# microsoft/OmniParser

Hardware: AMD Instinct MI355X
Metric: screenshots/sec end-to-end (detect+caption) @1920x1080 (higher is better)
Workload: dtype f32 (split-f16x3 MFMA)

## Files before the change

include/omni_amd.h:

```cpp
#ifndef OMNI_AMD_H
#define OMNI_AMD_H

#include <stdint.h>
#include <stddef.h>

#ifdef __cplusplus
extern "C" {
#endif

#define OMNI_ABI_VERSION 3

enum { OMNI_F32 = 0, OMNI_F16 = 1 };
enum { OMNI_ACT_NONE = 0, OMNI_ACT_SILU = 1, OMNI_ACT_GELU = 2 };
enum {
  OMNI_OK = 0,
  OMNI_E_ARG = -1,
  OMNI_E_HIP = -2,
  OMNI_E_NODEV = -3
};

const char* omni_last_error(void);
int omni_abi_version(void);
int omni_device_count(void);
int omni_overflow_count(int reset, unsigned long long* count);

typedef struct omni_op {
  int32_t kind;
  int32_t dtype;
  void*   p[8];
  int32_t i[32];
  float   f[8];
} omni_op_t;

enum {
  OMNI_OP_CONV = 1,
  OMNI_OP_AVGPOOL2 = 2,
  OMNI_OP_MAXPOOL = 3,
  OMNI_OP_RESIZE_NEAREST = 4,
  OMNI_OP_LETTERBOX = 5,
  OMNI_OP_DETECT_DECODE = 6,
  OMNI_OP_NMS = 7,
  OMNI_OP_DWCONV3 = 8,
  OMNI_OP_LAYERNORM = 9,
  OMNI_OP_ATTN_ROWS = 10,
  OMNI_OP_CHAN_ATTN = 11,
  OMNI_OP_PROJ_PREP = 12,
  OMNI_OP_ASSEMBLE = 13,
  OMNI_OP_EMBED_STEP = 14,
  OMNI_OP_ATTN_DECODE = 15,
  OMNI_OP_GREEDY_STEP = 16,
  OMNI_OP_CROP_RESIZE = 17,
  OMNI_OP_DWCONV3_LN = 18,
  OMNI_OP_SPLIT_CONVERT = 19,
  OMNI_OP_GLUE = 20,
  OMNI_OP_OVERLAY = 21,
  OMNI_OP_PNG_PACK = 22,
  OMNI_OP_PNG_DEFLATE = 23,
  OMNI_OP_MLP_FUSED = 24,
  OMNI_OP_BEAM_STEP,
  OMNI_OP__COUNT,
  OMNI_OP_GREEDY_CTRL_STEP = OMNI_OP__COUNT,
  OMNI_OP_GREEDY_VOCAB_STEP = OMNI_OP_GREEDY_CTRL_STEP + 1,
  OMNI_OP_VISUAL_MATCH = OMNI_OP_GREEDY_VOCAB_STEP + 1,
  OMNI_OP_REGION_OCR = OMNI_OP_VISUAL_MATCH + 1,
  OMNI_OP__END
};

#define OMNI_OCR_CLASS_STRIP 1000
#define OMNI_OCR_CLASS_TEXT 1001
#define OMNI_OCR_CLASS_HARD 1002

#define OMNI_VOCAB_HEADER_BYTES 32
#define OMNI_VOCAB_MAX_NODES 65536
#define OMNI_VOCAB_MAX_LABEL 64
typedef struct omni_vocab_trie {
  int32_t n_nodes;
  int32_t n_edges;
  int32_t longest;
  int32_t reserved[5];
} omni_vocab_trie_t;

#define OMNI_GEN_CTRL_HEADER_BYTES 32
#define OMNI_GEN_CTRL_MAX_BAD 64
#define OMNI_GEN_CTRL_MAX_BAD_LEN 8
typedef struct omni_gen_ctrl {
  float penalty;
  int32_t ngram;
  int32_t min_new_tokens;
  int32_t begin_index;
  int32_t n_bad;
  int32_t bad_stride;
  int32_t reserved[2];
} omni_gen_ctrl_t;

typedef struct omni_cand {
  float x1, y1, x2, y2;
  float score;
  int32_t cls;
  int32_t anchor;
  int32_t pad;
} omni_cand_t;

int omni_op_launch(const omni_op_t* op, void* stream);

typedef struct omni_plan omni_plan_t;
int omni_plan_create(const omni_op_t* ops, int n_ops, omni_plan_t** out);
int omni_plan_run(omni_plan_t* plan, void* stream);
int omni_plan_capture(omni_plan_t* plan, void* stream);
int omni_plan_replay(omni_plan_t* plan, void* stream);
int omni_plan_num_ops(const omni_plan_t* plan);
void omni_plan_destroy(omni_plan_t* plan);

int omni_resample_coeffs(int in_size, int out_size, int filter, int32_t* h_bounds, int32_t* h_coef);

int omni_plan_time(omni_plan_t* plan, void* stream, int iters, float* ms);

int omni_plan_profile(omni_plan_t* plan, void* stream, float* h_ms);

int omni_debug_tile_map(int mtiles, int ntiles, int xcd_n, long long weight_bytes, int bid, int* mt, int* nt, int* grid,
// ... 27 lines not shown
```

omniparser_amd/_lib.py:

```python
import ctypes
from ctypes import c_char_p, c_float, c_int, c_int32, c_void_p, POINTER, Structure

from . import build as _build


F32, F16 = 0, 1
ACT_NONE, ACT_SILU, ACT_GELU = 0, 1, 2
OP_CONV, OP_AVGPOOL2, OP_MAXPOOL, OP_RESIZE_NEAREST, OP_LETTERBOX, OP_DETECT_DECODE, OP_NMS = 1, 2, 3, 4, 5, 6, 7
OP_DWCONV3, OP_LAYERNORM, OP_ATTN_ROWS, OP_CHAN_ATTN, OP_PROJ_PREP, OP_ASSEMBLE = 8, 9, 10, 11, 12, 13
OP_EMBED_STEP, OP_ATTN_DECODE, OP_GREEDY_STEP, OP_CROP_RESIZE, OP_DWCONV3_LN, OP_SPLIT_CONVERT, OP_GLUE = 14, 15, 16, 17, 18, 19, 20
OP_OVERLAY, OP_PNG_PACK, OP_PNG_DEFLATE, OP_MLP_FUSED, OP_BEAM_STEP = 21, 22, 23, 24, 25
OP_GREEDY_CTRL_STEP = 26
OP_GREEDY_VOCAB_STEP = 27
OP_VISUAL_MATCH = 28
OP_REGION_OCR = 29
OCR_CLASS_STRIP, OCR_CLASS_TEXT, OCR_CLASS_HARD = 1000, 1001, 1002
CAND_BYTES = 32
ABI_VERSION = 3

EXPORTS = [
    "omni_last_error", "omni_abi_version", "omni_device_count", "omni_op_launch",
    "omni_plan_create", "omni_plan_run", "omni_plan_capture", "omni_plan_replay",
    "omni_plan_num_ops", "omni_plan_destroy", "omni_resample_coeffs", "omni_plan_time", "omni_debug_tile_map",
    "omni_debug_conv_cfg",
    "omni_plan_profile",
    "omni_model_load", "omni_model_destroy", "omni_model_int", "omni_model_tensor", "omni_model_run",
    "omni_detector_create", "omni_detector_infer", "omni_captioner_create", "omni_captioner_caption",
    "omni_overflow_count",
    "omni_visual_match_cfg",
]


class OmniOp(Structure):
    _fields_ = [
        ("kind", c_int32),
        ("dtype", c_int32),
        ("p", c_void_p * 8),
        ("i", c_int32 * 32),
        ("f", c_float * 8),
    ]


class OmniError(RuntimeError):
    pass


_lib = None


def lib():
    global _lib
    if _lib is not None:
        return _lib
    path = _build.ensure_built()
    import torch
    _lib = bind(path)
    return _lib


def bind(path):
    L = ctypes.CDLL(str(path))
    missing = [s for s in EXPORTS if not hasattr(L, s)]
    if missing:
        raise OmniError(f"{path} does not export {missing}")
    L.omni_last_error.restype = c_char_p
    L.omni_abi_version.restype = c_int
    L.omni_device_count.restype = c_int
    L.omni_op_launch.argtypes = [POINTER(OmniOp), c_void_p]
# ... 268 lines not shown
```

omniparser_amd/bundle.py:

```python
import bisect
import struct
from typing import Dict

import numpy as np
import torch

from . import _lib as L
from . import planner

MAGIC = b"OMNIPLN%d" % L.ABI_VERSION
ROLE = {"scratch": 0, "zero": 1, "const": 2}


def _name(s: str) -> bytes:
    b = s.encode()
    assert len(b) < 32, s
    return b.ljust(32, b"\0")


def f32_bits(x: float) -> int:
    return struct.unpack("<i", struct.pack("<f", float(x)))[0]


def write_bundle(path, plans: Dict[str, list], named: Dict[str, tuple], ints: Dict[str, int]):
# ... 88 lines not shown
        ops = []
        for _ in range(n):
            kind, dtype = struct.unpack_from("<ii", b, p); p += 8
            ptrs = [struct.unpack_from("<iq", b, p + 12 * j) for j in range(8)]; p += 96
            ii = struct.unpack_from("<32i", b, p); p += 128
            ff = struct.unpack_from("<8f", b, p); p += 32
            ops.append((kind, dtype, ptrs, ii, ff))
        plans[nm] = ops
    named = {}
    for _ in range(nn):
        nm = b[p:p + 32].rstrip(b"\0").decode(); p += 32
        named[nm] = struct.unpack_from("<iqq", b, p); p += 20
    ints = {}
    for _ in range(ni):
        nm = b[p:p + 32].rstrip(b"\0").decode(); p += 32
        (ints[nm],) = struct.unpack_from("<q", b, p); p += 8
    return {"tensors": tensors, "plans": plans, "named": named, "ints": ints}


def export_detector(det, iw: int, ih: int, path, imgsz=640, conf=0.05, iou=0.1, max_det=300, batch=1):
    dp = det.get_plan(iw, ih, imgsz, conf, iou, max_det, batch=batch)
    t = lambda x: (x, 0, x.numel() * x.element_size())
    named = {"img": t(dp.img), "out_boxes": t(dp.out_boxes), "out_scores": t(dp.out_scores), "out_cls": t(dp.out_cls),
             "out_count": t(dp.out_count)}
    ints = {"model": 1, "batch": batch, "img_w": iw, "img_h": ih, "max_det": max_det, "dtype": det.dtype}
    return write_bundle(path, {"detect": dp.plan.ops}, named, ints)


def export_captioner(cap, path, capacity=8, max_new_tokens=20):
    from .florence import CLIP_MEAN, CLIP_STD
    R = cap.resolution
    cp = cap.plans(capacity, R, max_new_tokens)
    pb = planner.PlanBuilder(cap.device, cap.dtype)
    lut = pb.upload(torch.from_numpy((np.arange(256).astype(np.float64) * (1 / 255)).astype(np.float32)))
    boxes = pb.raw((capacity, 4), torch.int32)
    c64 = pb.raw((capacity, 64, 64, 3), torch.uint8)
    t = lambda x: (x, 0, x.numel() * x.element_size())
    named = {"x_in": t(cp.x_in.t), "ids": t(cp.ids), "finished": t(cp.finished), "step": t(cp.step), "lut": t(lut), "boxes": t(boxes),
             "c64": t(c64),
             "vision_out": t(cp.vision_out.t), "enc_out": t(cp.enc_out.t), "logits": t(cp.logits.t)}
    ks = 0
    if R != 64:
        b, k = L.resample_coeffs(64, R, 1)
        bb, kk = pb.upload(torch.from_numpy(b)), pb.upload(torch.from_numpy(k))
        tmp = pb.raw((capacity, 64, R, 3), torch.uint8)
        named.update(bic_bounds=t(bb), bic_coef=t(kk), tmp=t(tmp))
        ks = k.shape[1]
    cp._bundle_keep = pb.keep
    ints = {"model": 2, "capacity": capacity, "R": R, "T": cp.T, "max_new": max_new_tokens, "start_token": cp.start_token, "pad": cap.w.pad,
            "eos": cap.w.eos, "ksize": ks, "ldo": cp.x_in.ld, "dtype": cap.dtype}
    for j in range(3):
        ints[f"mean{j}"] = f32_bits(CLIP_MEAN[j])
        ints[f"std{j}"] = f32_bits(CLIP_STD[j])
    return write_bundle(path, {"encode": cp.encode_plan.ops, "step": cp.step_plan.ops}, named, ints)
```

omniparser_amd/csrc/capi.hip:

```cpp
#include "omni_internal.h"

#include <math.h>
#include <stdarg.h>
#include <stdlib.h>
#include <string.h>
#include <vector>

static thread_local char g_err[512] = "";

void omni_set_error(const char* fmt, ...) {
  va_list ap;
  va_start(ap, fmt);
  vsnprintf(g_err, sizeof(g_err), fmt, ap);
  va_end(ap);
}

extern "C" const char* omni_last_error(void) { return g_err; }
extern "C" int omni_abi_version(void) { return OMNI_ABI_VERSION; }

static omni_ovf_reader_t g_ovf_readers[8];
static int g_ovf_n = 0;
void omni_register_overflow_reader(omni_ovf_reader_t fn) {
  if (g_ovf_n < 8) g_ovf_readers[g_ovf_n++] = fn;
}
extern "C" int omni_overflow_count(int reset, unsigned long long* count) {
  OMNI_REQUIRE(count != nullptr, "omni_overflow_count: null result pointer");
  unsigned long long total = 0;
  for (int k = 0; k < g_ovf_n; ++k) {
    unsigned int v = 0;
    if (g_ovf_readers[k](&v, reset)) {
      omni_set_error("omni_overflow_count: reading the device counter failed");
      return OMNI_E_HIP;
    }
    total += v;
  }
  *count = total;
  return OMNI_OK;
}

extern "C" int omni_device_count(void) {
  int n = 0;
  hipError_t e = hipGetDeviceCount(&n);
  if (e != hipSuccess) {
    omni_set_error("hipGetDeviceCount: %s", hipGetErrorString(e));
    return OMNI_E_NODEV;
  }
  return n;
}

static int dispatch(const omni_op_t* op, hipStream_t s) {
  switch (op->kind) {
    case OMNI_OP_CONV: return op->i[20] == 2 ? omni_launch_gemm_dma(op, s) : omni_launch_conv(op, s);
    case OMNI_OP_SPLIT_CONVERT: return omni_launch_split_convert(op, s);
    case OMNI_OP_MLP_FUSED: return omni_launch_mlp_fused(op, s);
    case OMNI_OP_GLUE: return omni_launch_glue(op, s);
    case OMNI_OP_OVERLAY: return omni_launch_overlay(op, s);
    case OMNI_OP_PNG_PACK: return omni_launch_png_pack(op, s);
    case OMNI_OP_PNG_DEFLATE: return omni_launch_png_deflate(op, s);
    case OMNI_OP_AVGPOOL2: return omni_launch_avgpool2(op, s);
    case OMNI_OP_MAXPOOL: return omni_launch_maxpool(op, s);
    case OMNI_OP_RESIZE_NEAREST: return omni_launch_resize_nearest(op, s);
    case OMNI_OP_LETTERBOX: return omni_launch_letterbox(op, s);
    case OMNI_OP_DETECT_DECODE: return omni_launch_detect_decode(op, s);
    case OMNI_OP_NMS: return omni_launch_nms(op, s);
    case OMNI_OP_DWCONV3: return omni_launch_dwconv3(op, s);
    case OMNI_OP_LAYERNORM: return omni_launch_layernorm(op, s);
    case OMNI_OP_DWCONV3_LN: return omni_launch_dwconv3_ln(op, s);
    case OMNI_OP_ATTN_ROWS: case OMNI_OP_CHAN_ATTN: case OMNI_OP_ATTN_DECODE: return omni_launch_attention(op, s);
    case OMNI_OP_PROJ_PREP: case OMNI_OP_ASSEMBLE: case OMNI_OP_EMBED_STEP: case OMNI_OP_GREEDY_STEP:
    case OMNI_OP_BEAM_STEP: case OMNI_OP_GREEDY_CTRL_STEP: case OMNI_OP_CROP_RESIZE: return omni_launch_misc(op, s);
    case OMNI_OP_GREEDY_VOCAB_STEP: return omni_launch_vocab_step(op, s);
    case OMNI_OP_VISUAL_MATCH: return omni_launch_visual_match(op, s);
    case OMNI_OP_REGION_OCR: return omni_launch_region_ocr(op, s);
    default:
      omni_set_error("unknown op kind %d", op->kind);
      return OMNI_E_ARG;
  }
}

static bool check_ptrs_enabled() {
  const char* e = getenv("OMNI_CHECK_PTRS");
  if (e && e[0] == '0') return false;
  static const int ndev = [] { int n = 0; const bool ok = hipGetDeviceCount(&n) == hipSuccess; if (!ok) (void)hipGetLastError(); return ok ? n : 0; }();
  return ndev > 0;
}

static void op_extents(const omni_op_t* op, long long ext[8]) {
  for (int k = 0; k < 8; ++k) ext[k] = 1;
  const long long esz = op->dtype == OMNI_F32 ? 4 : 2;
  const int* i = op->i;
  auto span = [&](long long rows, long long ld, long long coff, long long c) { return rows > 0 ? ((rows - 1) * ld + coff + c) * esz : 1; };
  switch (op->kind) {
    case OMNI_OP_CONV: {
      const long long B = i[0], H = i[1], W = i[2], Cin = i[3], Cout = i[12], M = B * i[10] * i[11], K = (long long)i[6] * i[7] * Cin;
      ext[0] = span(B * H * W, i[4], i[5], i[25] ? i[4] : Cin);
      ext[1] = Cout * K * (i[20] ? 4 : esz);
      ext[2] = Cout * 4;
      ext[3] = span(M, i[16], i[17], Cout);
      ext[4] = span(M, i[13], i[14], Cout);
      ext[5] = i[19] > 0 ? (long long)i[19] * 1024 : 1;
      if (i[24] > 0) ext[6] = (long long)i[24] * 4;
      if (i[20] == 2 && i[26] > 0) {
        const long long nimg = (M + i[26] - 1) / i[26];
        ext[1] += (nimg - 1) * (long long)i[27];
        ext[6] = nimg * 4;
        if (i[29] == 1) ext[2] = nimg * Cout * 4;
      }
      if (i[20] == 2 && i[28] == 1) {
        ext[7] = (M / 256) * (Cout / 64) * 4096;
        ext[4] = 1;
      }
      break;
    }
    case OMNI_OP_CHAN_ATTN: {
      const long long B = i[0], N = i[1], C = i[3], G = i[4], ct = i[10] > 0 ? i[10] : (i[5] > 0 ? i[5] : 1);
      ext[0] = B * N * 3 * C * esz; ext[4] = B * N * C * esz; ext[5] = B * G * ((N + ct - 1) / ct) * 1024 * 4;
      if (i[8] == 1) { ext[1] = C * C * 4; ext[2] = ext[3] = B * C * C * 4; ext[6] = B * 4; ext[7] = B * (C / 64) * G * 4; }
      if (i[8] == 1 && i[11] == 1) { ext[1] += 2 * C * 4; ext[2] += B * C * 4; }
      break;
    }
    case OMNI_OP_BEAM_STEP: {
      const long long rows = (long long)i[0] * i[6], T = i[3];
      ext[0] = rows > 0 ? ((rows - 1) * i[2] + i[1]) * esz : 1;
      ext[1] = (long long)i[1] * 4;
      ext[2] = ext[4] = ext[5] = rows * T * 4;
      ext[3] = rows * 4;
      ext[7] = (long long)i[0] * (3LL * i[6] + 2) * 4;
      break;
    }
    case OMNI_OP_GREEDY_STEP:
      if (op->p[5] || op->p[7]) {
        const long long rows = i[0], T = i[3];
        ext[0] = rows > 0 ? ((rows - 1) * i[2] + i[1]) * esz : 1;
        ext[1] = (long long)i[1] * 4;
        ext[2] = ext[4] = ext[7] = rows * T * 4;
        ext[5] = rows * 4;
        ext[6] = 4;
      }
      break;
    case OMNI_OP_GREEDY_CTRL_STEP: {
      const long long rows = i[0], T = i[3];
      ext[0] = rows > 0 ? ((rows - 1) * i[2] + i[1]) * esz : 1;
      ext[1] = (long long)i[1] * 4;
      ext[2] = ext[4] = rows * T * 4;
      ext[3] = rows * 4;
      ext[6] = 4;
      ext[7] = i[12];
      break;
    }
    case OMNI_OP_GREEDY_VOCAB_STEP: {
      const long long rows = i[0], T = i[3];
      ext[0] = rows > 0 ? ((rows - 1) * i[2] + i[1]) * esz : 1;
      ext[1] = (long long)i[1] * 4;
      ext[2] = ext[4] = rows * T * 4;
      ext[3] = ext[5] = rows * 4;
      ext[6] = 4;
      ext[7] = i[12];
      break;
    }
    case OMNI_OP_VISUAL_MATCH: {
      const long long D = i[3];
      if (i[0] == 0) {
        ext[0] = i[1] > 0 ? (((long long)i[1] - 1) * i[2] + D) * esz : 1; ext[4] = (long long)i[1] * D * 4; ext[5] = (long long)i[1] * 4;
      } else if (const long long part = omni_visual_match_part_bytes(op)) {
        ext[5] = part;
        if (i[0] == 1) { ext[0] = (long long)i[1] * D * 4; ext[1] = (long long)i[2] * D * 4; }
// ... 40 lines not shown
      break;
    }
    case OMNI_OP_DETECT_DECODE: {
      for (int l = 0; l < 3; ++l) {
        const long long hw = (long long)(i[1] / (8 << l)) * (i[2] / (8 << l));
        ext[l] = span(hw, i[3 + l], i[13 + l], i[0]);
        ext[3 + l] = span(hw, i[6 + l], i[16 + l], i[12] ? 4 : 64);
      }
      ext[6] = (long long)i[9] * 32; ext[7] = 4;
      break;
    }
    case OMNI_OP_LAYERNORM: {
      const long long rows = (long long)i[0] * i[1], C = i[3];
      ext[0] = rows * C * esz; ext[1] = (long long)(i[5] > 0 ? i[5] : 1) * C * esz; ext[2] = C * 4; ext[3] = C * 4;
      ext[4] = rows * C * esz; ext[5] = rows * C * esz;
      break;
    }
    case OMNI_OP_DWCONV3: case OMNI_OP_DWCONV3_LN: {
      const long long n = (long long)i[0] * i[1] * i[2] * i[3] * esz, C = i[3];
      ext[0] = n; ext[1] = 9 * C * esz; ext[2] = C * 4; ext[4] = n;
      if (op->kind == OMNI_OP_DWCONV3_LN) { ext[3] = n; ext[5] = C * 4; ext[6] = C * 4; }
      break;
    }
    case OMNI_OP_ASSEMBLE: {
      const long long B = i[0], n_img = i[1], n_txt = i[2], C = i[3];
      ext[0] = B * n_img * C * esz; ext[1] = n_txt * C * esz; ext[2] = B * n_txt * 4; ext[3] = (long long)i[4] * C * esz;
      ext[4] = B * (n_img + n_txt) * C * esz;
      break;
    }
    case OMNI_OP_ATTN_ROWS:
      ext[7] = (long long)i[11] * 4;
      break;
    case OMNI_OP_ATTN_DECODE:
      ext[7] = i[7] > 0 ? (long long)((i[10] + (i[12] > 1 ? i[12] : 1) - 1) / (i[12] > 1 ? i[12] : 1)) * 4 : (long long)i[10] * i[8] * 4;
      break;
    case OMNI_OP_OVERLAY:
      if (op->p[3] || op->p[4] || i[3]) {
        const long long B = i[3] > 0 ? i[3] : 1;
        ext[0] = B * i[0] * i[1] * 3; ext[1] = (long long)i[2] * 32; ext[3] = B * 8; ext[4] = (B + 1) * 4;
      }
      break;
    case OMNI_OP_PNG_DEFLATE:
      if (i[5] == 2 && i[6] > 0 && i[0] > 0 && i[1] > 0) {
        const long long B = i[6], U = (long long)i[0] * (3LL * i[1] + 1), units = (U + 32767) / 32768;
        ext[0] = B * i[0] * i[1] * 3; ext[1] = B * i[2]; ext[2] = B * U; ext[3] = B * units * 33792; ext[4] = B * i[3] * 4;
        ext[5] = B * i[4] * 4; ext[6] = B * 4 * (((long long)i[2] + 2) / 3); ext[7] = B * units * 32768 * 4;
      }
      break;
    default: break;
  }
  for (int k = 0; k < 8; ++k) if (ext[k] < 1) ext[k] = 1;
}

static int check_op_ptrs(const omni_op_t* op, int index) {
  long long ext[8];
  op_extents(op, ext);
  for (int k = 0; k < 8; ++k) {
    const void* ptr = op->p[k];
    if (!ptr) continue;
    hipDeviceptr_t base = nullptr;
    size_t size = 0;
    hipError_t e = hipMemGetAddressRange(&base, &size, (hipDeviceptr_t)ptr);
    if (e != hipSuccess || !base) {
      (void)hipGetLastError();
      omni_set_error("op %d (kind %d): p[%d] = %p is not inside any device allocation (%s)", index, op->kind, k, ptr,
                     e != hipSuccess ? hipGetErrorString(e) : "no base");
      return OMNI_E_ARG;
    }
    const long long off = (const char*)ptr - (const char*)base;
    if (off < 0 || off + ext[k] > (long long)size) {
      omni_set_error("op %d (kind %d): p[%d] = %p + %lld bytes runs past its allocation [%p, +%zu)", index, op->kind, k, ptr, ext[k],
                     (void*)base, size);
      return OMNI_E_ARG;
    }
  }
  return OMNI_OK;
}

static int check_ctrl_block(const omni_op_t* op, int index) {
  if (op->kind != OMNI_OP_GREEDY_CTRL_STEP) return OMNI_OK;
  const long long bytes = op->i[12], nw = ((long long)op->i[1] + 31) >> 5, fixed = OMNI_GEN_CTRL_HEADER_BYTES + 8 * nw;
  if (!op->p[7] || op->i[1] <= 0 || bytes < fixed) {
    omni_set_error("op %d (greedy_ctrl_step): a control block of %lld bytes (i12) at p7 = %p cannot hold the header and two bitmaps over a "
                   "vocabulary of %d (%lld bytes)", index, bytes, op->p[7], op->i[1], fixed);
    return OMNI_E_ARG;
  }
  omni_gen_ctrl_t h;
  hipError_t e = hipMemcpy(&h, op->p[7], sizeof h, hipMemcpyDeviceToHost);
  if (e != hipSuccess) {
    (void)hipGetLastError();
    omni_set_error("op %d (greedy_ctrl_step): the header of the control block p7 = %p cannot be read (%s)", index, op->p[7], hipGetErrorString(e));
    return OMNI_E_ARG;
  }
  if (h.n_bad < 0 || h.n_bad > OMNI_GEN_CTRL_MAX_BAD || (h.n_bad > 0 && (h.bad_stride < 3 || h.bad_stride > OMNI_GEN_CTRL_MAX_BAD_LEN + 1))) {
    omni_set_error("op %d (greedy_ctrl_step): the control block claims %d bad-word sequences of stride %d (at most %d of 2..%d tokens)", index,
                   h.n_bad, h.bad_stride, OMNI_GEN_CTRL_MAX_BAD, OMNI_GEN_CTRL_MAX_BAD_LEN);
    return OMNI_E_ARG;
  }
  const long long need = fixed + 4LL * h.n_bad * h.bad_stride;
  if (bytes < need) {
    omni_set_error("op %d (greedy_ctrl_step): the control block's header claims %d bad-word sequences of stride %d = %lld bytes, i12 says %lld",
                   index, h.n_bad, h.bad_stride, need, bytes);
    return OMNI_E_ARG;
  }
  return OMNI_OK;
}

static int check_trie_block(const omni_op_t* op, int index) {
  if (op->kind != OMNI_OP_GREEDY_VOCAB_STEP) return OMNI_OK;
  const long long bytes = op->i[12];
  if (!op->p[7] || bytes < OMNI_VOCAB_HEADER_BYTES + 4) {
    omni_set_error("op %d (greedy_vocab_step): a trie block of %lld bytes (i12) at p7 = %p cannot hold the header and one node (%d bytes)",
                   index, bytes, op->p[7], OMNI_VOCAB_HEADER_BYTES + 4);
    return OMNI_E_ARG;
  }
  omni_vocab_trie_t h;
  hipError_t e = hipMemcpy(&h, op->p[7], sizeof h, hipMemcpyDeviceToHost);
  if (e != hipSuccess) {
    (void)hipGetLastError();
    omni_set_error("op %d (greedy_vocab_step): the header of the trie block p7 = %p cannot be read (%s)", index, op->p[7], hipGetErrorString(e));
    return OMNI_E_ARG;
  }
  if (h.n_nodes < 1 || h.n_nodes > OMNI_VOCAB_MAX_NODES || h.n_edges < 0 || h.n_edges >= h.n_nodes) {
    omni_set_error("op %d (greedy_vocab_step): the trie block claims %d nodes and %d edges (1..%d nodes, fewer edges than nodes)", index,
                   h.n_nodes, h.n_edges, OMNI_VOCAB_MAX_NODES);
    return OMNI_E_ARG;
  }
  const long long need = OMNI_VOCAB_HEADER_BYTES + 4LL * (h.n_nodes + 1 + 2LL * h.n_edges);
// ... 192 lines not shown
```

omniparser_amd/csrc/conv_igemm.hip:

```cpp
#include "omni_internal.h"
#include "gemm_common.h"
#include <stdlib.h>
#include <string.h>
#include <type_traits>

OMNI_RANGE_GUARD_TU()

namespace {

struct ConvArgs {
  const void* x; const void* w; const float* bias; const void* res; void* y;
  int B, H, W, Cin, ldi, in_coff, KH, KW, stride, pad, Ho, Wo;
  int Cout, ldo, out_coff, act, ldr, res_coff;
  int M, K, ktiles, cin_tiles;
  int splits, kt_per_split, mtiles, ntiles, xcd_order, xcd_n;
  float* ws;
  int* cnt;
  float scale;
  int vec_px;
};


template <typename T, int ACT, typename GetAcc>
__device__ __forceinline__ void epilogue_tile(const ConvArgs& a, int mb, int n, bool nok, float bias, GetAcc get) {
  if (!nok) return;
  T* __restrict__ Yb = reinterpret_cast<T*>(a.y) + (long long)mb * a.ldo + a.out_coff + n;
  const T* __restrict__ Rb = a.res ? reinterpret_cast<const T*>(a.res) + (long long)mb * a.ldr + a.res_coff + n : nullptr;
  float r[16];
#pragma unroll
  for (int e = 0; e < 16; ++e) {
    const int dm = (e & 3) + 8 * (e >> 2);
    r[e] = (Rb && mb + dm < a.M) ? ElemTraits<T>::to_f32(Rb[dm * a.ldr]) : 0.0f;
  }
  const float scale = a.scale;
  float amax = 0.0f;
#pragma unroll
  for (int e = 0; e < 16; ++e) {
    const int dm = (e & 3) + 8 * (e >> 2);
    float v = get(e) + bias;
    if (scale != 0.0f) v *= scale;
    if constexpr (ACT == OMNI_ACT_SILU) v = v / (1.0f + expf(-v));
    else if constexpr (ACT == OMNI_ACT_GELU) v = omni_gelu(v);
    v += r[e];
    if (mb + dm < a.M) {
      Yb[dm * a.ldo] = ElemTraits<T>::from_f32(v);
      amax = __builtin_fmaxf(__builtin_fabsf(v), amax);
    }
  }
  if constexpr (sizeof(T) == 4) omni_report_range(amax);
}

template <typename T, int BM, int BN, int RB, bool ALIGNED, bool PW>
__global__ __launch_bounds__(256) void conv_igemm_kernel(ConvArgs a) {
  constexpr int V = ElemTraits<T>::kVec;
  constexpr int VPR = RB / 16;
  constexpr int BKE = VPR * V;
  constexpr int ROWB = RB + 16;
  constexpr int RPP = 256 / VPR;
  constexpr int A_IT = BM / RPP;
  constexpr int B_IT = BN / RPP;
  constexpr int TM = BM / 64;
  constexpr int TN = BN / 64;
  constexpr int STAGE = (BM + BN) * ROWB;

  __shared__ __attribute__((aligned(16))) unsigned char lds[2 * STAGE];

  const int tid = threadIdx.x;
  const int lane = tid & 63;
  const int wave = tid >> 6;
  const int wm = wave >> 1, wn = wave & 1;
  int mt, nt;
  if (!tile_of_block(blockIdx.x, a.mtiles, a.ntiles, a.xcd_order, a.xcd_n, mt, nt)) return;
// ... 219 lines not shown
  if constexpr (sizeof(T) == 4) omni_report_range(__builtin_fabsf(v));
  reinterpret_cast<T*>(a.y)[m * a.ldo + a.out_coff + n] = ElemTraits<T>::from_f32(v);
}


__device__ __forceinline__ void split_f16x4(const u32x4& raw, uint2& hi, uint2& lo) {
  typedef __fp16 hv2 __attribute__((ext_vector_type(2)));
  f32x4 v = __builtin_bit_cast(f32x4, raw);
  hv2 h01 = __builtin_amdgcn_cvt_pkrtz(v[0], v[1]);
  hv2 h23 = __builtin_amdgcn_cvt_pkrtz(v[2], v[3]);
  float r0 = (v[0] - (float)h01[0]) * 2048.0f, r1 = (v[1] - (float)h01[1]) * 2048.0f;
  float r2 = (v[2] - (float)h23[0]) * 2048.0f, r3 = (v[3] - (float)h23[1]) * 2048.0f;
  hv2 l01 = __builtin_amdgcn_cvt_pkrtz(r0, r1);
  hv2 l23 = __builtin_amdgcn_cvt_pkrtz(r2, r3);
  hi.x = __builtin_bit_cast(unsigned, h01); hi.y = __builtin_bit_cast(unsigned, h23);
  lo.x = __builtin_bit_cast(unsigned, l01); lo.y = __builtin_bit_cast(unsigned, l23);
}

#ifndef OMNI_AGENT_ST_F32
#define OMNI_AGENT_ST_F32(p, v) __hip_atomic_store((p), (v), __ATOMIC_RELAXED, __HIP_MEMORY_SCOPE_AGENT)
#define OMNI_AGENT_LD_F32(p) __hip_atomic_load((p), __ATOMIC_RELAXED, __HIP_MEMORY_SCOPE_AGENT)
#define OMNI_AGENT_ADD_I32(p, v) __hip_atomic_fetch_add((p), (v), __ATOMIC_RELAXED, __HIP_MEMORY_SCOPE_AGENT)
#define OMNI_AGENT_ST_I32(p, v) __hip_atomic_store((p), (v), __ATOMIC_RELAXED, __HIP_MEMORY_SCOPE_AGENT)
#endif

__device__ __forceinline__ void combine_partials(const ConvArgs& a, int mb, int n, bool nok, float* sum) {
#pragma unroll
  for (int e = 0; e < 16; ++e) sum[e] = 0.0f;
  if (!nok) return;
  const int total = a.M * a.Cout;
  int off[16];
#pragma unroll
  for (int e = 0; e < 16; ++e) {
    const int m = mb + (e & 3) + 8 * (e >> 2);
    off[e] = (m < a.M ? m : a.M - 1) * a.Cout + n;
  }
  const float* __restrict__ base = a.ws;
  int z = 0;
  for (; z + 2 <= a.splits; z += 2, base += 2 * (long long)total) {
    float v0[16], v1[16];
#pragma unroll
    for (int e = 0; e < 16; ++e) v0[e] = OMNI_AGENT_LD_F32(base + off[e]);
#pragma unroll
    for (int e = 0; e < 16; ++e) v1[e] = OMNI_AGENT_LD_F32(base + total + off[e]);
#pragma unroll
    for (int e = 0; e < 16; ++e) sum[e] = (sum[e] + v0[e]) + v1[e];
  }
  if (z < a.splits) {
#pragma unroll
    for (int e = 0; e < 16; ++e) sum[e] += OMNI_AGENT_LD_F32(base + off[e]);
  }
}

template <int BM, int BN, int NW, bool PW>
__global__ __launch_bounds__(NW * 64, 2) void conv_split_kernel(ConvArgs a) {
  constexpr int RB = 128, ROWB = RB + 16, VPR = 8, RPP = NW * 8;
  constexpr int BKE = 32;
  constexpr int A_IT = BM / RPP, B_IT = BN / RPP;
  constexpr int WN = NW / 2;
  constexpr int TM = BM / 64, TN = BN / (32 * WN);
  constexpr int STAGE = (BM + BN) * ROWB;
  __shared__ __attribute__((aligned(16))) unsigned char lds[2 * STAGE];

  const int tid = threadIdx.x, lane = tid & 63, wave = tid >> 6;
  const int wm = wave / WN, wn = wave % WN;
  int mt, nt;
  if (!tile_of_block(blockIdx.x, a.mtiles, a.ntiles, a.xcd_order, a.xcd_n, mt, nt)) return;
  const int m0 = mt * BM, n0 = nt * BN;
  const int vec = tid % VPR, r0 = tid / VPR;
  const int kt0 = blockIdx.z * a.kt_per_split;
  const int kt1 = min(kt0 + a.kt_per_split, a.ktiles);

  const float* __restrict__ X = reinterpret_cast<const float*>(a.x);
  const unsigned char* __restrict__ Wb = reinterpret_cast<const unsigned char*>(a.w);

  long long a_base[A_IT];
  int a_hi0[A_IT], a_wi0[A_IT];
  bool a_ok[A_IT];
  const float* a_row[A_IT];
#pragma unroll
  for (int it = 0; it < A_IT; ++it) {
    int m = m0 + r0 + it * RPP;
    a_ok[it] = m < a.M;
    int mm = a_ok[it] ? m : 0;
    int wo = mm % a.Wo;
    int t = mm / a.Wo;
    int ho = t % a.Ho;
    int b = t / a.Ho;
    a_hi0[it] = ho * a.stride - a.pad;
    a_wi0[it] = wo * a.stride - a.pad;
    a_base[it] = (long long)b * a.H * a.W * a.ldi + a.in_coff;
    a_row[it] = X + (long long)mm * a.ldi + a.in_coff + vec * 4;
  }
  const unsigned char* b_ptr[B_IT];
  bool b_ok[B_IT];
#pragma unroll
  for (int it = 0; it < B_IT; ++it) {
    int n = n0 + r0 + it * RPP;
    b_ok[it] = n < a.Cout;
    b_ptr[it] = Wb + (long long)(b_ok[it] ? n : 0) * a.K * 4 + vec * 16;
  }
  int w_r = 0, w_s = 0, w_c = 0;
  if (!PW) {
    int tap = kt0 / a.cin_tiles;
    w_c = (kt0 - tap * a.cin_tiles) * BKE;
    w_r = tap / a.KW;
    w_s = tap - w_r * a.KW;
// ... 39 lines not shown
      *reinterpret_cast<u32x4*>(sB + (r0 + it * RPP) * ROWB + vec * 16) = rb[it];
  };

  f32x16 accM[TM][TN], accC[TM][TN];
#pragma unroll
  for (int i = 0; i < TM; ++i)
#pragma unroll
    for (int j = 0; j < TN; ++j)
#pragma unroll
      for (int e = 0; e < 16; ++e) { accM[i][j][e] = 0.0f; accC[i][j][e] = 0.0f; }

  const int a_rd = (wm * (BM / 2) + (lane & 31)) * ROWB + (lane >> 5) * 16;
  const int b_rd = BM * ROWB + (wn * (BN / WN) + (lane & 31)) * ROWB + (lane >> 5) * 16;

  auto compute = [&](int stage) {
    const unsigned char* st = lds + stage * STAGE;
#pragma unroll
    for (int j16 = 0; j16 < 2; ++j16) {
      f16x8 ah[TM], al[TM], bh[TN], bl[TN];
#pragma unroll
      for (int i = 0; i < TM; ++i) {
        ah[i] = *reinterpret_cast<const f16x8*>(st + a_rd + i * 32 * ROWB + j16 * 64);
        al[i] = *reinterpret_cast<const f16x8*>(st + a_rd + i * 32 * ROWB + j16 * 64 + 32);
      }
#pragma unroll
      for (int j = 0; j < TN; ++j) {
        bh[j] = *reinterpret_cast<const f16x8*>(st + b_rd + j * 32 * ROWB + j16 * 64);
        bl[j] = *reinterpret_cast<const f16x8*>(st + b_rd + j * 32 * ROWB + j16 * 64 + 32);
      }
#pragma unroll
      for (int i = 0; i < TM; ++i)
#pragma unroll
        for (int j = 0; j < TN; ++j) {
          accM[i][j] = __builtin_amdgcn_mfma_f32_32x32x16_f16(ah[i], bh[j], accM[i][j], 0, 0, 0);
          accC[i][j] = __builtin_amdgcn_mfma_f32_32x32x16_f16(ah[i], bl[j], accC[i][j], 0, 0, 0);
          accC[i][j] = __builtin_amdgcn_mfma_f32_32x32x16_f16(al[i], bh[j], accC[i][j], 0, 0, 0);
        }
    }
  };

  if (kt0 < kt1) { load_tile(kt0, ra0, rb0); store_tile(0, ra0, rb0); }
  __syncthreads();
  int cur = 0;
  for (int kt = kt0; kt < kt1; ++kt) {
    const bool more = kt + 1 < kt1;
    if (more) load_tile(kt + 1, ra0, rb0);
    compute(cur);
    if (more) store_tile(cur ^ 1, ra0, rb0);
    __syncthreads();
    cur ^= 1;
  }

  const float inv = 1.0f / 2048.0f;
  if (a.splits > 1) {
    float* __restrict__ P = a.ws + (long long)blockIdx.z * a.M * a.Cout;
    const bool combine = a.cnt != nullptr;
#pragma unroll
    for (int j = 0; j < TN; ++j) {
      int n = n0 + wn * (BN / WN) + j * 32 + (lane & 31);
      if (n >= a.Cout) continue;
#pragma unroll
      for (int i = 0; i < TM; ++i) {
        int mb = m0 + wm * (BM / 2) + i * 32 + 4 * (lane >> 5);
#pragma unroll
        for (int e = 0; e < 16; ++e) {
          int m = mb + (e & 3) + 8 * (e >> 2);
          if (m < a.M) {
            const float v = accM[i][j][e] + accC[i][j][e] * inv;
            if (combine) OMNI_AGENT_ST_F32(&P[(long long)m * a.Cout + n], v);
            else P[(long long)m * a.Cout + n] = v;
          }
        }
      }
    }
    if (!combine) return;
    OMNI_WAIT_VMCNT(0);
    __syncthreads();
    int* const flag = reinterpret_cast<int*>(lds);
    if (tid == 0) *flag = OMNI_AGENT_ADD_I32(&a.cnt[mt * a.ntiles + nt], 1);
    __syncthreads();
    if (*flag != a.splits - 1) return;
    if (tid == 0) OMNI_AGENT_ST_I32(&a.cnt[mt * a.ntiles + nt], 0);
    auto fin = [&](auto tag) {
      constexpr int ACT = decltype(tag)::value;
#pragma unroll
      for (int j = 0; j < TN; ++j) {
        const int n = n0 + wn * (BN / WN) + j * 32 + (lane & 31);
        const bool nok = n < a.Cout;
        const float bias = (nok && a.bias) ? a.bias[n] : 0.0f;
#pragma unroll
        for (int i = 0; i < TM; ++i) {
          const int mb = m0 + wm * (BM / 2) + i * 32 + 4 * (lane >> 5);
          float sum[16];
          combine_partials(a, mb, n, nok, sum);
          epilogue_tile<float, ACT>(a, mb, n, nok, bias, [&](int e) { return sum[e]; });
        }
      }
    };
    if (a.act == OMNI_ACT_SILU) fin(std::integral_constant<int, OMNI_ACT_SILU>{});
    else if (a.act == OMNI_ACT_GELU) fin(std::integral_constant<int, OMNI_ACT_GELU>{});
    else fin(std::integral_constant<int, OMNI_ACT_NONE>{});
    return;
  }
  auto run = [&](auto tag) {
    constexpr int ACT = decltype(tag)::value;
#pragma unroll
    for (int j = 0; j < TN; ++j) {
      const int n = n0 + wn * (BN / WN) + j * 32 + (lane & 31);
      const bool nok = n < a.Cout;
      const float bias = (nok && a.bias) ? a.bias[n] : 0.0f;
#pragma unroll
      for (int i = 0; i < TM; ++i)
        epilogue_tile<float, ACT>(a, m0 + wm * (BM / 2) + i * 32 + 4 * (lane >> 5), n, nok, bias,
                                  [&](int e) { return accM[i][j][e] + accC[i][j][e] * inv; });
    }
  };
  if (a.act == OMNI_ACT_SILU) run(std::integral_constant<int, OMNI_ACT_SILU>{});
  else if (a.act == OMNI_ACT_GELU) run(std::integral_constant<int, OMNI_ACT_GELU>{});
  else run(std::integral_constant<int, OMNI_ACT_NONE>{});
}

enum { CONV_FAMILY_F32 = 0, CONV_FAMILY_F16 = 1, CONV_FAMILY_SPLIT = 2 };
enum { CONV_LOADER_GENERIC = 0, CONV_LOADER_ALIGNED = 1, CONV_LOADER_POINTWISE = 2, CONV_LOADER_ROW_PATCH = 3 };
struct ConvPlan {
  int family, bm, bn, rb, loader, waves;
};

template <int BM, int BN>
void launch_split_cfg(ConvArgs& a, const ConvPlan& p, hipStream_t s) {
  a.mtiles = (a.M + BM - 1) / BM;
  a.ntiles = (a.Cout + BN - 1) / BN;
  a.xcd_order = (a.mtiles >= 64 && a.ntiles > 1) ? 1 : 0;
  a.xcd_n = a.xcd_order ? choose_xcd_n(a.ntiles, 4ll * a.Cout * a.K) : 1;
  dim3 grid(tile_grid(a.mtiles, a.ntiles, a.xcd_order, a.xcd_n), 1, a.splits);
  const bool pw = p.loader == CONV_LOADER_POINTWISE;
  if constexpr (BM == 128 && BN == 128) {
    if (pw) hipLaunchKernelGGL((conv_split_kernel<BM, BN, 8, true>), grid, dim3(512), 0, s, a);
    else hipLaunchKernelGGL((conv_split_kernel<BM, BN, 8, false>), grid, dim3(512), 0, s, a);
  } else {
    if (pw) hipLaunchKernelGGL((conv_split_kernel<BM, BN, 4, true>), grid, dim3(256), 0, s, a);
    else hipLaunchKernelGGL((conv_split_kernel<BM, BN, 4, false>), grid, dim3(256), 0, s, a);
  }
  if (a.splits > 1 && !a.cnt) {
    long long total = (long long)a.M * a.Cout;
    hipLaunchKernelGGL((splitk_reduce_kernel<float>), dim3((unsigned)((total + 255) / 256)), dim3(256), 0, s, a);
  }
}

int plan_split(ConvArgs& a, long long ws_bytes, int force_tile, int force_splits, int* cnt, int n_cnt, ConvPlan& p) {
  a.cin_tiles = a.Cin / 32;
  a.ktiles = a.K / 32;
  int bn = a.Cout > 64 ? 128 : 64, bm = 128;
  auto blocks = [&](int m, int n) { return (long long)((a.M + m - 1) / m) * ((a.Cout + n - 1) / n); };
  if (blocks(bm, bn) < 512 && bn == 128) bn = 64;
  if (blocks(bm, bn) < 512) bm = 64;
  if (force_tile) {
    OMNI_REQUIRE(force_tile >= 1 && force_tile <= 3, "conv: bad tile code %d (1 = 64x64, 2 = 128x64, 3 = 128x128)", force_tile);
    bm = force_tile == 1 ? 64 : 128;
    bn = force_tile == 3 ? 128 : 64;
  }
  long long nb = blocks(bm, bn);
  a.splits = 1;
  const long long cap = a.ws ? ws_bytes / ((long long)a.M * a.Cout * 4) : 1;
  if (force_splits) {
    OMNI_REQUIRE(force_splits >= 1 && force_splits <= 64, "conv: bad split count %d", force_splits);
    a.splits = force_splits > a.ktiles ? a.ktiles : force_splits;
    if (a.splits > cap) a.splits = (int)(cap < 1 ? 1 : cap);
  } else if (nb < 512 && a.ws) {
    int want = (int)((768 + nb - 1) / nb);
    int maxs = a.ktiles / 4;
    if (maxs > 32) maxs = 32;
    if (maxs > cap) maxs = (int)cap;
    a.splits = want < maxs ? want : maxs;
    if (a.splits < 2) a.splits = 1;
  }
  a.kt_per_split = (a.ktiles + a.splits - 1) / a.splits;
  a.splits = (a.ktiles + a.kt_per_split - 1) / a.kt_per_split;
  a.cnt = (a.splits > 1 && cnt && nb <= n_cnt) ? cnt : nullptr;
  const bool pw = !a.vec_px && a.KH == 1 && a.KW == 1 && a.stride == 1 && a.pad == 0 && a.H == a.Ho && a.W == a.Wo;
  p.family = CONV_FAMILY_SPLIT;
  p.bm = bm; p.bn = bn; p.rb = 128;
  p.loader = a.vec_px ? CONV_LOADER_ROW_PATCH : pw ? CONV_LOADER_POINTWISE : CONV_LOADER_ALIGNED;
  p.waves = (bm == 128 && bn == 128) ? 8 : 4;
  return OMNI_OK;
}

template <typename T, int BM, int BN, int RB>
int launch_cfg(ConvArgs& a, const ConvPlan& p, hipStream_t s) {
  a.mtiles = (a.M + BM - 1) / BM;
  a.ntiles = (a.Cout + BN - 1) / BN;
// ... 41 lines not shown
    a.splits = want < maxs ? want : maxs;
    if (a.splits < 2) a.splits = 1;
  }
  a.kt_per_split = (a.ktiles + a.splits - 1) / a.splits;
  a.splits = (a.ktiles + a.kt_per_split - 1) / a.kt_per_split;
  a.cnt = nullptr;
  const bool pw = aligned && a.KH == 1 && a.KW == 1 && a.stride == 1 && a.pad == 0 && a.H == a.Ho && a.W == a.Wo;
  p.family = V == 4 ? CONV_FAMILY_F32 : CONV_FAMILY_F16;
  p.bm = bm; p.bn = bn; p.rb = rb;
  p.loader = pw ? CONV_LOADER_POINTWISE : aligned ? CONV_LOADER_ALIGNED : CONV_LOADER_GENERIC;
  p.waves = 4;
  return OMNI_OK;
}

template <typename T>
int launch_typed(ConvArgs& a, const ConvPlan& p, hipStream_t s) {
  if (p.rb == 128) return launch_cfg<T, 64, 64, 128>(a, p, s);
  if (p.bm == 128 && p.bn == 128) return launch_cfg<T, 128, 128, 64>(a, p, s);
  if (p.bm == 128 && p.bn == 64) return launch_cfg<T, 128, 64, 64>(a, p, s);
  return launch_cfg<T, 64, 64, 64>(a, p, s);
}

int plan_conv(const omni_op_t* op, ConvArgs& a, ConvPlan& p) {
  a.x = op->p[0]; a.w = op->p[1]; a.bias = (const float*)op->p[2]; a.res = op->p[3]; a.y = op->p[4];
  a.B = op->i[0]; a.H = op->i[1]; a.W = op->i[2]; a.Cin = op->i[3]; a.ldi = op->i[4]; a.in_coff = op->i[5];
  a.KH = op->i[6]; a.KW = op->i[7]; a.stride = op->i[8]; a.pad = op->i[9]; a.Ho = op->i[10]; a.Wo = op->i[11];
  a.Cout = op->i[12]; a.ldo = op->i[13]; a.out_coff = op->i[14]; a.act = op->i[15];
  a.ldr = op->i[16]; a.res_coff = op->i[17];
  a.scale = op->f[0];
  a.ws = (float*)op->p[5];
  const long long ws_bytes = a.ws ? (long long)op->i[19] * 1024 : 0;
  a.splits = 1; a.kt_per_split = 0;
  const int V = op->dtype == OMNI_F32 ? 4 : 8;
  OMNI_REQUIRE(op->dtype == OMNI_F32 || op->dtype == OMNI_F16, "conv: bad dtype %d", op->dtype);
  OMNI_REQUIRE(a.x && a.w && a.y, "conv: null pointer");
  OMNI_REQUIRE(a.B > 0 && a.H > 0 && a.W > 0 && a.Cin > 0 && a.Cout > 0 && a.Ho > 0 && a.Wo > 0, "conv: bad shape");
  OMNI_REQUIRE(a.Cin % V == 0 && a.ldi % V == 0 && a.in_coff % V == 0,
               "conv: Cin/ldi/in_coff (%d/%d/%d) must be multiples of %d", a.Cin, a.ldi, a.in_coff, V);
  OMNI_REQUIRE(a.KH > 0 && a.KW > 0 && a.stride > 0 && a.pad >= 0, "conv: bad window");
  OMNI_REQUIRE(a.act >= 0 && a.act <= OMNI_ACT_GELU, "conv: bad act %d", a.act);
  long long M = (long long)a.B * a.Ho * a.Wo;
  OMNI_REQUIRE(M < (1ll << 31), "conv: M too large");
  a.M = (int)M;
  a.K = a.KH * a.KW * a.Cin;
  a.vec_px = 0;
  if (op->i[25]) {
    OMNI_REQUIRE(op->i[25] == 1 && op->i[20] == 1 && a.KW == 1 && a.Cin == 32 && a.ldi == 4 && a.in_coff == 0 && a.KH <= 8,
                 "conv: row-patch mode (i25) needs i20 = 1, KW = 1, Cin = 32 (8 pixels of 4 channels), ldi = 4, in_coff = 0, KH <= 8");
    a.vec_px = 1;
  }
  if (op->i[20]) {
    OMNI_REQUIRE(op->dtype == OMNI_F32 && a.Cin % 32 == 0, "conv: split-f16 mode needs f32 activations and Cin %% 32 == 0");
    OMNI_REQUIRE(op->i[24] >= 0 && (op->i[24] == 0 || op->p[6]), "conv: i24 arrival counters without p6");
    return plan_split(a, ws_bytes, op->i[22], op->i[23], op->i[24] > 0 ? (int*)op->p[6] : nullptr, op->i[24], p);
  }
  return plan_typed(a, V, ws_bytes, op->i[22], p);
}

}

int omni_launch_conv(const omni_op_t* op, hipStream_t s) {
  ConvArgs a{};
  ConvPlan p{};
  int rc = plan_conv(op, a, p);
  if (rc) return rc;
  if (p.family == CONV_FAMILY_SPLIT) {
    if (p.bm == 128 && p.bn == 128) launch_split_cfg<128, 128>(a, p, s);
    else if (p.bm == 128 && p.bn == 64) launch_split_cfg<128, 64>(a, p, s);
    else launch_split_cfg<64, 64>(a, p, s);
  } else {
    rc = p.family == CONV_FAMILY_F32 ? launch_typed<float>(a, p, s) : launch_typed<half_t>(a, p, s);
    if (rc) return rc;
  }
  OMNI_HIP_CHECK(hipGetLastError());
  return OMNI_OK;
}

extern "C" int omni_debug_conv_cfg(const omni_op_t* op, int out[8]) {
  OMNI_REQUIRE(op && out, "omni_debug_conv_cfg: null argument");
  OMNI_REQUIRE(op->kind == OMNI_OP_CONV && op->i[20] != 2, "omni_debug_conv_cfg: not a register-staged conv op (kind %d, i20 = %d)", op->kind, op->i[20]);
  ConvArgs a{};
  ConvPlan p{};
  int rc = plan_conv(op, a, p);
  if (rc) return rc;
  out[0] = p.family; out[1] = p.bm; out[2] = p.bn; out[3] = p.rb; out[4] = p.loader; out[5] = a.splits;
  out[6] = a.splits > 1 ? (a.cnt ? 2 : 1) : 0;
  out[7] = p.waves;
  return OMNI_OK;
}

extern "C" int omni_debug_tile_map(int mtiles, int ntiles, int xcd_n, long long weight_bytes, int bid, int* mt, int* nt, int* grid,
                                   int* xcd_n_used) {
  if (mtiles <= 0 || ntiles <= 0 || !mt || !nt) return OMNI_E_ARG;
  const int xcd_order = (mtiles >= 64 && ntiles > 1) ? 1 : 0;
  int xn = xcd_order ? (weight_bytes >= 0 ? choose_xcd_n(ntiles, weight_bytes) : xcd_n) : 1;
  if (xn != 1 && xn != 2 && xn != 4 && xn != 8) return OMNI_E_ARG;
  if (ntiles % xn) return OMNI_E_ARG;
  if (grid) *grid = (int)tile_grid(mtiles, ntiles, xcd_order, xn);
  if (xcd_n_used) *xcd_n_used = xn;
  int a = -1, b = -1;
  bool ok = tile_of_block(bid, mtiles, ntiles, xcd_order, xn, a, b);
  *mt = ok ? a : -1;
  *nt = ok ? b : -1;
  return OMNI_OK;
}
```

omniparser_amd/csrc/gemm_dma.hip:

```cpp
#include "omni_internal.h"
#include "gemm_common.h"
#include <string.h>
#include <type_traits>

OMNI_RANGE_GUARD_TU()

namespace {

typedef __attribute__((address_space(3))) void lds_void;

struct GemmArgs {
  const unsigned char* x; const unsigned char* w; const float* bias; const float* res; unsigned char* y;
  int M, N, K, nk;
  int ldi, in_coff, ldo, out_coff, ldr, res_coff;
  int mtiles, ntiles, xcd_order, xcd_n;
  float oscale;
  int img_tiles; unsigned w_img_stride; const float* img_oscale;
  int bias_img_stride;
};

constexpr int GEMM_EPI_SCORES = 3;

#if defined(__AMDGCN__)
struct RowBuf {
  __amdgpu_buffer_rsrc_t r;
  __device__ __forceinline__ RowBuf(const void* base, unsigned bytes) : r(__builtin_amdgcn_make_buffer_rsrc((void*)base, 0, (int)bytes, 0x00020000)) {}
  __device__ __forceinline__ void store16(unsigned off, f32x4 v) const { __builtin_amdgcn_raw_buffer_store_b128(__builtin_bit_cast(u32x4, v), r, (int)off, 0, 0); }
  __device__ __forceinline__ f32x4 load16(unsigned off) const { return __builtin_bit_cast(f32x4, __builtin_amdgcn_raw_buffer_load_b128(r, (int)off, 0, 0)); }
};
#else
struct RowBuf {
  unsigned char* base; unsigned bytes;
  RowBuf(const void* b, unsigned n) : base((unsigned char*)b), bytes(n) {}
  void store16(unsigned off, f32x4 v) const { if (off + 16u <= bytes) *reinterpret_cast<f32x4*>(base + off) = v; }
  f32x4 load16(unsigned off) const { return off + 16u <= bytes ? *reinterpret_cast<const f32x4*>(base + off) : f32x4{0.f, 0.f, 0.f, 0.f}; }
};
#endif

template <int BM, int BN, int WM, int WN, int TM, int TN, int LDS_BYTES, int ACT, bool OSPLIT, bool RES>
__device__ __forceinline__ void gemm_epilogue(f32x16 (&acc)[TM][TN], const GemmArgs& a, const float* bias, unsigned char* lds, int m0, int n0, int wave,
                                              int lane, float osc) {
  constexpr int NW = WM * WN;
  const int wm = wave / WN, wn = wave % WN;
  const int hsel = lane >> 5;
  static_assert(TN % 2 == 0, "epilogue stages 64 channels (256 bytes per row) of a wave at a time");
  constexpr int EP = 272;
  static_assert(NW * 32 * EP <= LDS_BYTES, "epilogue staging must fit the LDS ring");
  __syncthreads();
  unsigned char* stg = lds + wave * (32 * EP);
  float amax = 0.0f;
  const int rrow = lane >> 4, chunk = lane & 15;
  const int trows = min(a.M - m0, BM), wc0 = n0 + wn * (BN / WN);
  const RowBuf ybuf(a.y + ((long long)m0 * a.ldo + a.out_coff + wc0) * 4, (unsigned)(trows - 1) * (unsigned)(a.ldo * 4) + (BN / WN) * 4);
  const RowBuf rbuf(RES ? reinterpret_cast<const unsigned char*>(a.res) + ((long long)m0 * a.ldr + a.res_coff + wc0) * 4 : a.y,
                    RES ? (unsigned)(trows - 1) * (unsigned)(a.ldr * 4) + (BN / WN) * 4 : 0u);
  const unsigned yoff = (unsigned)(wm * (BM / WM) + rrow) * (unsigned)(a.ldo * 4) + chunk * 16;
  const unsigned roff = (unsigned)(wm * (BM / WM) + rrow) * (unsigned)(a.ldr * 4) + chunk * 16;
  static_assert(!(RES && OSPLIT), "residual + format-B output is not a layer of this model");
#pragma unroll
  for (int jh = 0; jh < TN / 2; ++jh) {
    const int nw0 = n0 + wn * (BN / WN) + jh * 64;
    f32x4 bq[2][4];
#pragma unroll
    for (int j = 0; j < 2; ++j)
#pragma unroll
      for (int q = 0; q < 4; ++q)
        bq[j][q] = bias ? *reinterpret_cast<const f32x4*>(bias + nw0 + 4 * hsel + j * 32 + q * 8) : f32x4{0.f, 0.f, 0.f, 0.f};
    f32x4 rres[8];
    auto load_res = [&](int i) {
#pragma unroll
      for (int it = 0; it < 8; ++it) rres[it] = rbuf.load16(roff + (unsigned)(i * 32 + it * 4) * (unsigned)(a.ldr * 4) + jh * 256);
    };
    if constexpr (RES) load_res(0);
#pragma unroll
    for (int i = 0; i < TM; ++i) {
      unsigned char* wr = stg + (lane & 31) * EP;
#pragma unroll
      for (int j = 0; j < 2; ++j)
#pragma unroll
        for (int q = 0; q < 4; ++q) {
          const f32x16& ac = acc[i][jh * 2 + j];
          float v[4];
          if constexpr (ACT == OMNI_ACT_GELU) {
#pragma unroll
            for (int c = 0; c < 4; c += 2) {
              const f32x2 g = omni_gelu2(__builtin_elementwise_fma(f32x2{ac[q * 4 + c], ac[q * 4 + c + 1]}, (f32x2)osc, f32x2{bq[j][q][c], bq[j][q][c + 1]}));
              v[c] = g[0]; v[c + 1] = g[1];
            }
          } else {
#pragma unroll
            for (int c = 0; c < 4; c += 2) {
              f32x2 t = __builtin_elementwise_fma(f32x2{ac[q * 4 + c], ac[q * 4 + c + 1]}, (f32x2)osc, f32x2{bq[j][q][c], bq[j][q][c + 1]});
              if constexpr (ACT == OMNI_ACT_SILU) t = f32x2{t[0] / (1.0f + expf(-t[0])), t[1] / (1.0f + expf(-t[1]))};
              v[c] = t[0]; v[c + 1] = t[1];
            }
          }
          const int cl = j * 32 + q * 8 + 4 * hsel;
          if constexpr (OSPLIT) {
            uint2 hi, lo;
            omni_split4(v, hi, lo, amax);
            *reinterpret_cast<uint2*>(wr + omni_split_off(cl)) = hi;
            *reinterpret_cast<uint2*>(wr + omni_split_off(cl) + 32) = lo;
          } else {
            *reinterpret_cast<f32x4*>(wr + cl * 4) = f32x4{v[0], v[1], v[2], v[3]};
          }
        }
      OMNI_WAVE_SYNC();
// ... 233 lines not shown
  };
  if constexpr (SCHED == 2) {
    static_assert(BM == 256 && BN == 256 && WM == 2 && WN == 4 && NSTAGE == 2 && TM == 4 && TN == 2 && A_DMA == 4 && B_DMA == 4, "ping-pong: 256x256 tile, 8 waves");
    OMNI_WAIT_VMCNT(0);
    __builtin_amdgcn_s_barrier();
    if (wm == 1) __builtin_amdgcn_s_barrier();
    auto phase_barrier = [&]() {
      __builtin_amdgcn_sched_barrier(0);
      __builtin_amdgcn_s_barrier();
      __builtin_amdgcn_sched_barrier(0);
    };
    {
      AF afp;
      auto slice_pp = [&](int kt, auto more_tag) {
        constexpr bool MORE = decltype(more_tag)::value;
        const unsigned char* st = lds + stage * STAGE;
#pragma unroll
        for (int u = 0; u < 4; ++u) {
          const int g = u & 1, ip = u >> 1;
          if (u < 2) loadW(st, g, wf[g]);
          loadA(st, g, ip, afp);
          if constexpr (MORE) {
            if (u == 0) { issue_piece(kt + 1, nstage, 0); issue_piece(kt + 1, nstage, 2); }
            if (u == 1) { issue_piece(kt + 1, nstage, A_DMA + 0); issue_piece(kt + 1, nstage, A_DMA + 1); }
            if (u == 2) { issue_piece(kt + 1, nstage, A_DMA + 2); issue_piece(kt + 1, nstage, A_DMA + 3); }
            if (u == 3) { issue_piece(kt + 1, nstage, 1); issue_piece(kt + 1, nstage, 3); }
            if (u == 1) OMNI_WAIT_VMCNT(4);
            if (u == 3) OMNI_WAIT_VMCNT(2);
          } else {
            if (u == 1) OMNI_WAIT_VMCNT(0);
          }
          phase_barrier();
          __builtin_amdgcn_s_setprio(1);
          mma(afp, wf[g], ip);
          __builtin_amdgcn_s_setprio(0);
          phase_barrier();
        }
        stage ^= 1;
        nstage ^= 1;
      };
      int ktp = 0;
      for (; ktp + 1 < nk; ++ktp) slice_pp(ktp, std::true_type{});
      for (; ktp < nk; ++ktp) slice_pp(ktp, std::false_type{});
    }
    if (wm == 0) __builtin_amdgcn_s_barrier();
  } else {
  int kt = 0;
  for (; kt + NSTAGE - 1 < nk; ++kt) slice(kt, std::true_type{});
  for (; kt < nk; ++kt) slice(kt, std::false_type{});
  }

  if constexpr (ACT == GEMM_EPI_SCORES)
    gemm_scores_epilogue<BM, BN, WM, WN, TM, TN, NSTAGE * STAGE>(acc, a, lds, img, __builtin_amdgcn_readfirstlane(mt) - img * a.img_tiles, n0, wave, lane, osc);
  else
    gemm_epilogue<BM, BN, WM, WN, TM, TN, NSTAGE * STAGE, ACT, OSPLIT, RES>(acc, a, a.bias + (long long)img * a.bias_img_stride, lds, m0, n0, wave,
                                                                            lane, osc);
#endif
}

__global__ __launch_bounds__(256) void split_convert_kernel(const float* __restrict__ x, unsigned char* __restrict__ y, long long rows,
                                                            int C, int ldi, int in_coff, int ldo, int out_coff) {
  const int gpr = C / 16;
  const long long idx = (long long)blockIdx.x * blockDim.x + threadIdx.x;
  if (idx >= rows * gpr) return;
  const long long r = idx / gpr;
  const int g = (int)(idx - r * gpr);
  const float* src = x + r * ldi + in_coff + g * 16;
  f32x4 v[4];
#pragma unroll
  for (int q = 0; q < 4; ++q) v[q] = *reinterpret_cast<const f32x4*>(src + q * 4);
  uint2 hi[4], lo[4];
#pragma unroll
  for (int q = 0; q < 4; ++q) {
    float t[4] = {v[q][0], v[q][1], v[q][2], v[q][3]};
    omni_split4(t, hi[q], lo[q]);
  }
  unsigned char* dst = y + (r * ldo + out_coff + g * 16) * 4;
  *reinterpret_cast<u32x4*>(dst) = u32x4{hi[0].x, hi[0].y, hi[1].x, hi[1].y};
  *reinterpret_cast<u32x4*>(dst + 16) = u32x4{hi[2].x, hi[2].y, hi[3].x, hi[3].y};
  *reinterpret_cast<u32x4*>(dst + 32) = u32x4{lo[0].x, lo[0].y, lo[1].x, lo[1].y};
  *reinterpret_cast<u32x4*>(dst + 48) = u32x4{lo[2].x, lo[2].y, lo[3].x, lo[3].y};
}

struct MlpArgs {
  const unsigned char* x; const unsigned char* w1; const unsigned char* w2; const float* b1;
  GemmArgs ep{};
  int ldi, in_coff;
  float osc1;
};

template <int C, int HID>
__global__ __launch_bounds__(256, 2) void mlp_fused_kernel(MlpArgs a) {
#if defined(__HIP_DEVICE_COMPILE__)
  static_assert(C == 128 && HID % 32 == 0, "written for the C = 128 stage: 8 K groups in registers, 4 output tiles");
  constexpr int NW = 4, KG = C / 16, OB = C / 32, NCH = HID / 32;
  constexpr int W1B = 32 * C * 4, W2B = C * 128, STAGE = W1B + W2B;
  constexpr int P1 = W1B / 1024 / NW, P2 = W2B / 1024 / NW;
  __shared__ __attribute__((aligned(16))) unsigned char lds[2 * STAGE + HID * 4];
  float* lb1 = reinterpret_cast<float*>(lds + 2 * STAGE);

  const int tid = threadIdx.x, lane = tid & 63;
  const int wave = __builtin_amdgcn_readfirstlane(tid >> 6);
  const int m0 = blockIdx.x * (NW * 32);
  const int hsel = lane >> 5, swz = (lane >> 1) & 7;

  for (int e = tid * 4; e < HID; e += 256 * 4) *reinterpret_cast<f32x4*>(lb1 + e) = *reinterpret_cast<const f32x4*>(a.b1 + e);

  const int rsub = lane >> 3, slot = lane & 7;
  unsigned voff1[P1], voff2[P2];
// ... 51 lines not shown
    if (c + 1 < NCH) issue(c + 1, stage ^ 1);
    const unsigned char* st = lds + stage * STAGE;
    f32x16 a1[2];
#pragma unroll
    for (int e = 0; e < 16; ++e) { a1[0][e] = 0.0f; a1[1][e] = 0.0f; }
#pragma unroll
    for (int g = 0; g < KG; g += 2) {
      const unsigned char* sl = st + (g >> 1) * 4096;
      const f16x8 wh0 = *reinterpret_cast<const f16x8*>(sl + fo[0][0]), wl0 = *reinterpret_cast<const f16x8*>(sl + fo[0][1]);
      const f16x8 wh1 = *reinterpret_cast<const f16x8*>(sl + fo[1][0]), wl1 = *reinterpret_cast<const f16x8*>(sl + fo[1][1]);
      a1[0] = __builtin_amdgcn_mfma_f32_32x32x16_f16(wh0, xh[g], a1[0], 0, 0, 0);
      a1[1] = __builtin_amdgcn_mfma_f32_32x32x16_f16(wh1, xh[g + 1], a1[1], 0, 0, 0);
      a1[0] = __builtin_amdgcn_mfma_f32_32x32x16_f16(wl0, xh[g], a1[0], 0, 0, 0);
      a1[1] = __builtin_amdgcn_mfma_f32_32x32x16_f16(wl1, xh[g + 1], a1[1], 0, 0, 0);
      a1[0] = __builtin_amdgcn_mfma_f32_32x32x16_f16(wh0, xl[g], a1[0], 0, 0, 0);
      a1[1] = __builtin_amdgcn_mfma_f32_32x32x16_f16(wh1, xl[g + 1], a1[1], 0, 0, 0);
    }
    f16x8 gh[2], gl[2];
#pragma unroll
    for (int kg = 0; kg < 2; ++kg) {
      uint2 hq[2], lq[2];
#pragma unroll
      for (int qq = 0; qq < 2; ++qq) {
        const int q = kg * 2 + qq;
        const f32x4 bq = *reinterpret_cast<const f32x4*>(lb1 + c * 32 + 8 * q + 4 * hsel);
        float v[4];
#pragma unroll
        for (int r = 0; r < 4; r += 2) {
          const f32x2 t = omni_gelu2(__builtin_elementwise_fma(f32x2{a1[0][q * 4 + r], a1[0][q * 4 + r + 1]} + f32x2{a1[1][q * 4 + r], a1[1][q * 4 + r + 1]},
                                                               (f32x2)osc1, f32x2{bq[r], bq[r + 1]}));
          v[r] = t[0]; v[r + 1] = t[1];
        }
        omni_split4(v, hq[qq], lq[qq], amax);
      }
      gh[kg] = __builtin_bit_cast(f16x8, u32x4{hq[0].x, hq[0].y, hq[1].x, hq[1].y});
      gl[kg] = __builtin_bit_cast(f16x8, u32x4{lq[0].x, lq[0].y, lq[1].x, lq[1].y});
    }
#pragma unroll
    for (int kg = 0; kg < 2; ++kg)
#pragma unroll
      for (int j = 0; j < OB; j += 2) {
        const unsigned char* sw = st + W1B + j * 4096;
        const f16x8 wh0 = *reinterpret_cast<const f16x8*>(sw + fo[kg][0]), wl0 = *reinterpret_cast<const f16x8*>(sw + fo[kg][1]);
        const f16x8 wh1 = *reinterpret_cast<const f16x8*>(sw + 4096 + fo[kg][0]), wl1 = *reinterpret_cast<const f16x8*>(sw + 4096 + fo[kg][1]);
        acc2[0][j] = __builtin_amdgcn_mfma_f32_32x32x16_f16(wh0, gh[kg], acc2[0][j], 0, 0, 0);
        acc2[0][j + 1] = __builtin_amdgcn_mfma_f32_32x32x16_f16(wh1, gh[kg], acc2[0][j + 1], 0, 0, 0);
        acc2[0][j] = __builtin_amdgcn_mfma_f32_32x32x16_f16(wl0, gh[kg], acc2[0][j], 0, 0, 0);
        acc2[0][j + 1] = __builtin_amdgcn_mfma_f32_32x32x16_f16(wl1, gh[kg], acc2[0][j + 1], 0, 0, 0);
        acc2[0][j] = __builtin_amdgcn_mfma_f32_32x32x16_f16(wh0, gl[kg], acc2[0][j], 0, 0, 0);
        acc2[0][j + 1] = __builtin_amdgcn_mfma_f32_32x32x16_f16(wh1, gl[kg], acc2[0][j + 1], 0, 0, 0);
      }
  }
  omni_report_range(amax);
  gemm_epilogue<NW * 32, C, NW, 1, 1, OB, 2 * STAGE, OMNI_ACT_NONE, false, true>(acc2, a.ep, a.ep.bias, lds, m0, 0, wave, lane, a.ep.oscale);
#endif
}

template <int BM, int BN, int WM, int WN, int NSTAGE>
int launch_tile(GemmArgs& a, int rows_per_img, int act, int osplit, bool scores, hipStream_t s) {
  if (rows_per_img % BM != 0) {
    omni_set_error("gemm_dma: per-image weights need whole %d-row tiles per image (rows per image %d)", BM, rows_per_img);
    return OMNI_E_ARG;
  }
  a.img_tiles = rows_per_img / BM;
  a.mtiles = (a.M + BM - 1) / BM;
  a.ntiles = a.N / BN;
  a.xcd_order = (a.mtiles >= 64 && a.ntiles > 1) ? 1 : 0;
  a.xcd_n = a.xcd_order ? choose_xcd_n(a.ntiles, 4ll * a.N * a.K) : 1;
  dim3 grid(tile_grid(a.mtiles, a.ntiles, a.xcd_order, a.xcd_n)), block(WM * WN * 64);
  const bool res = a.res != nullptr;
  constexpr int SCHED1 = (BM == 256 && BN == 256) ? 1 : 0;
  const char* sched_e = getenv("OMNI_GEMM_SCHED");
  const bool lockstep = sched_e && atoi(sched_e) == 1;
#define OMNI_GD(ACT_, OS_, RES_)                                                                                                   \
  do {                                                                                                                             \
    if constexpr (BM == 256 && BN == 256) {                                                                                        \
      if (!lockstep) { hipLaunchKernelGGL((gemm_dma_kernel<BM, BN, WM, WN, NSTAGE, ACT_, OS_, RES_, 2>), grid, block, 0, s, a); break; }  \
    }                                                                                                                              \
    hipLaunchKernelGGL((gemm_dma_kernel<BM, BN, WM, WN, NSTAGE, ACT_, OS_, RES_, SCHED1>), grid, block, 0, s, a);                  \
  } while (0)
  if (scores) {
    if constexpr (BM == 256 && BN == 256) OMNI_GD(GEMM_EPI_SCORES, false, false);
    else { omni_set_error("gemm_dma: the scores epilogue is built for the 256x256 tile"); return OMNI_E_ARG; }
  }
  else if (act == OMNI_ACT_NONE && !osplit && !res) OMNI_GD(OMNI_ACT_NONE, false, false);
  else if (act == OMNI_ACT_NONE && !osplit && res) OMNI_GD(OMNI_ACT_NONE, false, true);
  else if (act == OMNI_ACT_NONE && osplit && !res) OMNI_GD(OMNI_ACT_NONE, true, false);
  else if (act == OMNI_ACT_GELU && osplit && !res) OMNI_GD(OMNI_ACT_GELU, true, false);
  else if (act == OMNI_ACT_GELU && !osplit && !res) OMNI_GD(OMNI_ACT_GELU, false, false);
#undef OMNI_GD
  else {
    omni_set_error("gemm_dma: unsupported epilogue (act %d, split out %d, residual %d)", act, osplit, (int)res);
    return OMNI_E_ARG;
  }
  return OMNI_OK;
}

}

int omni_launch_gemm_dma(const omni_op_t* op, hipStream_t s) {
  GemmArgs a{};
  a.x = (const unsigned char*)op->p[0]; a.w = (const unsigned char*)op->p[1]; a.bias = (const float*)op->p[2];
  a.res = (const float*)op->p[3]; a.y = (unsigned char*)op->p[4];
  const int B = op->i[0], H = op->i[1], W = op->i[2];
  a.K = op->i[3]; a.ldi = op->i[4]; a.in_coff = op->i[5];
  a.N = op->i[12]; a.ldo = op->i[13]; a.out_coff = op->i[14];
  const int act = op->i[15];
  a.ldr = op->i[16]; a.res_coff = op->i[17];
  const int osplit = op->i[21];
  a.oscale = op->f[1] != 0.0f ? op->f[1] : 1.0f;
  OMNI_REQUIRE(op->dtype == OMNI_F32, "gemm_dma: f32 plans only");
  OMNI_REQUIRE(op->i[28] == 0 || op->i[28] == 1, "gemm_dma: unknown epilogue mode %d (i28)", op->i[28]);
  const bool scores = op->i[28] == 1;
  OMNI_REQUIRE(a.x && a.w && (a.y || scores), "gemm_dma: null pointer");
  if (scores) a.y = (unsigned char*)op->p[7];
  OMNI_REQUIRE(op->i[6] == 1 && op->i[7] == 1 && op->i[8] == 1 && op->i[9] == 0 && op->i[10] == H && op->i[11] == W,
               "gemm_dma: pointwise layers only");
  OMNI_REQUIRE(op->f[0] == 0.0f, "gemm_dma: output scale is not supported");
  const long long M = (long long)B * H * W;
  OMNI_REQUIRE(M > 0 && M < (1ll << 31), "gemm_dma: bad M");
  a.M = (int)M;
  OMNI_REQUIRE(a.K >= 32 && a.K % 32 == 0 && a.N % 128 == 0, "gemm_dma: needs K %% 32 == 0 and N %% 128 == 0 (K %d, N %d)", a.K, a.N);
  OMNI_REQUIRE(a.ldi % 16 == 0 && a.in_coff % 16 == 0, "gemm_dma: split input needs 16-channel aligned ld / offset (%d, %d)", a.ldi, a.in_coff);
  OMNI_REQUIRE(a.ldo % 4 == 0 && a.out_coff % 4 == 0 && (!osplit || (a.ldo % 16 == 0 && a.out_coff % 16 == 0)), "gemm_dma: output alignment");
  OMNI_REQUIRE(!a.res || (a.ldr % 4 == 0 && a.res_coff % 4 == 0), "gemm_dma: residual alignment");
  OMNI_REQUIRE((long long)a.ldi * 4 * 256 < (1ll << 31) && (long long)a.K * 4 * 256 < (1ll << 31) && (long long)a.ldo * 4 * 256 < (1ll << 31) &&
               (long long)a.ldr * 4 * 256 < (1ll << 31), "gemm_dma: row stride too large");
  a.nk = a.K / 32;
  const int rows_per_img = op->i[26];
  OMNI_REQUIRE(rows_per_img >= 0 && op->i[27] >= 0, "gemm_dma: bad per-image weight arguments (%d rows, stride %d)", rows_per_img, op->i[27]);
  if (rows_per_img > 0) {
    OMNI_REQUIRE(a.M % rows_per_img == 0, "gemm_dma: %d rows are no whole number of images of %d rows", a.M, rows_per_img);
    OMNI_REQUIRE(op->i[27] % 16 == 0 && (op->i[27] == 0 || op->i[27] >= a.N * a.K * 4), "gemm_dma: per-image weight stride %d (N %d, K %d)", op->i[27], a.N, a.K);
    a.w_img_stride = (unsigned)op->i[27];
    a.img_oscale = (const float*)op->p[6];
  }
  OMNI_REQUIRE(op->i[29] == 0 || op->i[29] == 1, "gemm_dma: unknown bias mode %d (i29)", op->i[29]);
  if (op->i[29] == 1) {
    OMNI_REQUIRE(rows_per_img > 0 && op->i[28] == 0, "gemm_dma: a per-image bias (i29) needs per-image mode (i26 > 0) and no scores epilogue");
    OMNI_REQUIRE(a.bias && (uintptr_t)a.bias % 16 == 0, "gemm_dma: the per-image bias table (p2) must be a 16-byte aligned pointer");
    a.bias_img_stride = a.N;
  }
  if (scores) {
    OMNI_REQUIRE(a.y, "gemm_dma: the scores epilogue needs its workspace (p7)");
    OMNI_REQUIRE(rows_per_img > 0 && rows_per_img % 256 == 0, "gemm_dma: the scores epilogue needs whole 256-row chunks per image (i26 = %d)", rows_per_img);
    OMNI_REQUIRE(a.N % 256 == 0, "gemm_dma: the scores epilogue needs N %% 256 == 0 (N %d)", a.N);
    OMNI_REQUIRE(act == OMNI_ACT_NONE && !a.res && !osplit, "gemm_dma: the scores epilogue takes no activation, residual or format-B output");
  }
  int tile = (a.N % 256 == 0) ? 0 : 1;
  {
    const long long mt256 = (a.M + 255) / 256;
    if (mt256 * (a.N / (tile == 0 ? 256 : 128)) < 256) tile = (tile == 0 && mt256 * (a.N / 128) >= 256) ? 1 : 2;
  }
  if (rows_per_img > 0 && rows_per_img % 256 != 0) tile = 2;
  if (const char* e = getenv("OMNI_GEMM_TILE")) {
    if (!strcmp(e, "256x128")) tile = 1;
    else if (!strcmp(e, "128x128")) tile = 2;
    else if (!strcmp(e, "256x256") && a.N % 256 == 0) tile = 0;
  }
  if (scores) tile = 0;
  int rc;
  if (tile == 0) rc = launch_tile<256, 256, 2, 4, 2>(a, rows_per_img, act, osplit, scores, s);
  else if (tile == 1) rc = launch_tile<256, 128, 4, 2, 3>(a, rows_per_img, act, osplit, false, s);
  else rc = launch_tile<128, 128, 2, 2, 2>(a, rows_per_img, act, osplit, false, s);
  if (rc) return rc;
  OMNI_HIP_CHECK(hipGetLastError());
  return OMNI_OK;
}

int omni_launch_split_convert(const omni_op_t* op, hipStream_t s) {
  OMNI_REQUIRE(op->i[6] == 0 || op->i[6] == 1, "split_convert: unknown mode %d (i6)", op->i[6]);
  if (op->i[6] == 1) return omni_launch_chan_repack(op, s);
  const long long rows = (long long)op->i[0] * (op->i[1] > 0 ? op->i[1] : 1);
  const int C = op->i[3], ldi = op->i[4], in_coff = op->i[5], ldo = op->i[13], out_coff = op->i[14];
  OMNI_REQUIRE(op->dtype == OMNI_F32 && op->p[0] && op->p[4], "split_convert: f32 plans, non-null pointers");
  OMNI_REQUIRE(rows > 0 && C > 0 && C % 16 == 0 && ldi % 16 == 0 && in_coff % 16 == 0 && ldo % 16 == 0 && out_coff % 16 == 0,
               "split_convert: 16-channel alignment (C %d, ld %d/%d, off %d/%d)", C, ldi, ldo, in_coff, out_coff);
  const long long total = rows * (C / 16);
  hipLaunchKernelGGL(split_convert_kernel, dim3((unsigned)((total + 255) / 256)), dim3(256), 0, s, (const float*)op->p[0],
                     (unsigned char*)op->p[4], rows, C, ldi, in_coff, ldo, out_coff);
  OMNI_HIP_CHECK(hipGetLastError());
  return OMNI_OK;
}

int omni_launch_mlp_fused(const omni_op_t* op, hipStream_t s) {
  MlpArgs a{};
  a.x = (const unsigned char*)op->p[0]; a.w1 = (const unsigned char*)op->p[1]; a.b1 = (const float*)op->p[2];
  a.w2 = (const unsigned char*)op->p[5];
  a.ep.x = nullptr; a.ep.w = nullptr; a.ep.bias = (const float*)op->p[6]; a.ep.res = (const float*)op->p[3]; a.ep.y = (unsigned char*)op->p[4];
  const long long M = (long long)op->i[0] * (op->i[1] > 0 ? op->i[1] : 1);
  const int C = op->i[3], HID = op->i[12];
  a.ldi = op->i[4]; a.in_coff = op->i[5];
  a.ep.ldo = op->i[13]; a.ep.out_coff = op->i[14]; a.ep.ldr = op->i[16]; a.ep.res_coff = op->i[17];
  a.osc1 = op->f[1] != 0.0f ? op->f[1] : 1.0f;
  a.ep.oscale = op->f[2] != 0.0f ? op->f[2] : 1.0f;
  OMNI_REQUIRE(op->dtype == OMNI_F32, "mlp_fused: f32 plans only");
  OMNI_REQUIRE(a.x && a.w1 && a.w2 && a.b1 && a.ep.bias && a.ep.res && a.ep.y, "mlp_fused: null pointer (both biases and the residual are required)");
  OMNI_REQUIRE(C == 128 && HID == 512, "mlp_fused: built for C = 128, hidden = 512 (got %d, %d)", C, HID);
  OMNI_REQUIRE(M > 0 && M < (1ll << 31), "mlp_fused: bad row count");
  OMNI_REQUIRE(a.ldi % 16 == 0 && a.in_coff % 16 == 0, "mlp_fused: split input needs 16-channel aligned ld / offset");
  OMNI_REQUIRE(a.ep.ldo % 4 == 0 && a.ep.out_coff % 4 == 0 && a.ep.ldr % 4 == 0 && a.ep.res_coff % 4 == 0, "mlp_fused: output / residual alignment");
  OMNI_REQUIRE((long long)a.ep.ldo * 4 * 128 < (1ll << 31) && (long long)a.ep.ldr * 4 * 128 < (1ll << 31), "mlp_fused: row stride too large");
  a.ep.M = (int)M; a.ep.N = C; a.ep.K = HID; a.ep.nk = 0; a.ep.ldi = 0; a.ep.in_coff = 0;
  a.ep.mtiles = a.ep.ntiles = a.ep.xcd_order = a.ep.xcd_n = 0;
  hipLaunchKernelGGL((mlp_fused_kernel<128, 512>), dim3((unsigned)((M + 127) / 128)), dim3(256), 0, s, a);
  OMNI_HIP_CHECK(hipGetLastError());
  return OMNI_OK;
}
```

omniparser_amd/csrc/omni_internal.h:

```cpp
#pragma once
#include <hip/hip_runtime.h>
#include <hip/hip_fp16.h>
#include <stdint.h>
#include <stdio.h>
#include <string>
#include "../../include/omni_amd.h"

void omni_set_error(const char* fmt, ...);

#define OMNI_HIP_CHECK(expr)                                                        \
  do {                                                                              \
    hipError_t _e = (expr);                                                         \
    if (_e != hipSuccess) {                                                         \
      omni_set_error("%s failed: %s (%s:%d)", #expr, hipGetErrorString(_e), __FILE__, __LINE__); \
      return OMNI_E_HIP;                                                            \
    }                                                                               \
  } while (0)

#define OMNI_REQUIRE(cond, ...)                 \
  do {                                          \
    if (!(cond)) {                              \
      omni_set_error(__VA_ARGS__);              \
      return OMNI_E_ARG;                        \
    }                                           \
// ... 90 lines not shown
  hv2 l = __builtin_amdgcn_cvt_pkrtz(v - (float)h[0], 0.0f);
  hi = (unsigned short)(__builtin_bit_cast(unsigned, h) & 0xffffu);
  lo = (unsigned short)(__builtin_bit_cast(unsigned, l) & 0xffffu);
}
__device__ __forceinline__ int omni_split_half_index(int c) { return (c >> 4) * 32 + (c & 15); }
__device__ __forceinline__ int omni_split_off(int c) { return (c >> 4) * 64 + (c & 15) * 2; }

__device__ __forceinline__ float omni_erff(float a) {
  const float t = __builtin_fminf(__builtin_fabsf(a), 6.0f), s = t * t;
  float r = __builtin_fmaf(-1.72853470e-5f, t, 3.83197126e-4f);
  const float u = __builtin_fmaf(-3.88396438e-3f, t, 2.42546219e-2f);
  r = __builtin_fmaf(r, s, u);
  r = __builtin_fmaf(r, t, -1.06777847e-1f);
  r = __builtin_fmaf(r, t, -6.34846687e-1f);
  r = __builtin_fmaf(r, t, -1.28717512e-1f);
  r = __builtin_fmaf(r, t, -t);
  const float big = __builtin_copysignf(1.0f - __expf(r), a);
  float q = -5.96761703e-4f;
  q = __builtin_fmaf(q, s, 4.99119423e-3f);
  q = __builtin_fmaf(q, s, -2.67681349e-2f);
  q = __builtin_fmaf(q, s, 1.12819925e-1f);
  q = __builtin_fmaf(q, s, -3.76125336e-1f);
  q = __builtin_fmaf(q, s, 1.28379166e-1f);
  const float small = __builtin_fmaf(q, a, a);
  return t > 0.927734375f ? big : small;
}
__device__ __forceinline__ float omni_gelu(float v) { return 0.5f * v * (1.0f + omni_erff(v * 0.70710678118654752440f)); }
typedef float f32x2 __attribute__((ext_vector_type(2)));
#if defined(__AMDGCN__)
#define OMNI_EXP2(x) __builtin_amdgcn_exp2f(x)
#else
#define OMNI_EXP2(x) __builtin_exp2f(x)
#endif
__device__ __forceinline__ f32x2 omni_gelu2(f32x2 v) {
  const f32x2 t = __builtin_elementwise_min(__builtin_elementwise_abs(v), (f32x2)8.48528137423857f);
  f32x2 p = __builtin_elementwise_fma((f32x2)1.137868688e-09f, t, (f32x2)-5.171069262e-08f);
  p = __builtin_elementwise_fma(p, t, (f32x2)1.014483701e-06f);
  p = __builtin_elementwise_fma(p, t, (f32x2)-1.117507963e-05f);
  p = __builtin_elementwise_fma(p, t, (f32x2)7.388171798e-05f);
  p = __builtin_elementwise_fma(p, t, (f32x2)-2.645340865e-04f);
  p = __builtin_elementwise_fma(p, t, (f32x2)-3.723767077e-05f);
  p = __builtin_elementwise_fma(p, t, (f32x2)6.994847674e-03f);
  p = __builtin_elementwise_fma(p, t, (f32x2)-5.247364566e-02f);
  p = __builtin_elementwise_fma(p, t, (f32x2)-4.592104554e-01f);
  p = __builtin_elementwise_fma(p, t, (f32x2)-1.151105404e+00f);
  p = __builtin_elementwise_fma(p, t, (f32x2)1.941864447e-08f);
  const f32x2 E = {OMNI_EXP2(p[0]), OMNI_EXP2(p[1])};
  const f32x2 c1 = __builtin_elementwise_copysign((f32x2)0.5f, v);
  return v * __builtin_elementwise_fma(-c1, E, 0.5f + c1);
}

int omni_launch_conv(const omni_op_t* op, hipStream_t s);
int omni_launch_gemm_dma(const omni_op_t* op, hipStream_t s);
int omni_launch_split_convert(const omni_op_t* op, hipStream_t s);
int omni_launch_chan_repack(const omni_op_t* op, hipStream_t s);
int omni_launch_mlp_fused(const omni_op_t* op, hipStream_t s);
int omni_launch_avgpool2(const omni_op_t* op, hipStream_t s);
int omni_launch_maxpool(const omni_op_t* op, hipStream_t s);
int omni_launch_resize_nearest(const omni_op_t* op, hipStream_t s);
int omni_launch_letterbox(const omni_op_t* op, hipStream_t s);
int omni_launch_detect_decode(const omni_op_t* op, hipStream_t s);
int omni_launch_nms(const omni_op_t* op, hipStream_t s);
int omni_launch_dwconv3(const omni_op_t* op, hipStream_t s);
int omni_launch_layernorm(const omni_op_t* op, hipStream_t s);
int omni_launch_dwconv3_ln(const omni_op_t* op, hipStream_t s);
int omni_launch_attention(const omni_op_t* op, hipStream_t s);
int omni_launch_misc(const omni_op_t* op, hipStream_t s);
int omni_launch_vocab_step(const omni_op_t* op, hipStream_t s);
int omni_launch_visual_match(const omni_op_t* op, hipStream_t s);
long long omni_visual_match_part_bytes(const omni_op_t* op);
int omni_launch_region_ocr(const omni_op_t* op, hipStream_t s);
bool omni_region_ocr_extents(const omni_op_t* op, long long ext[8]);
int omni_launch_glue(const omni_op_t* op, hipStream_t s);
int omni_launch_overlay(const omni_op_t* op, hipStream_t s);
int omni_launch_png_pack(const omni_op_t* op, hipStream_t s);
int omni_launch_png_deflate(const omni_op_t* op, hipStream_t s);
```

omniparser_amd/florence.py:

```python
import contextlib
import json
import math
import os
from pathlib import Path
from types import SimpleNamespace
from typing import Dict, List, Optional

import numpy as np
import torch

from . import _lib as L
from .planner import PlanBuilder, View, torch_dtype

PROMPT_IDS = [0, 2264, 473, 5, 2274, 6190, 116, 2]
TEXT_CAPACITIES = (8, 16, 32, 64)


def text_capacity(n_tokens: int) -> int:
    for c in TEXT_CAPACITIES:
        if n_tokens <= c:
            return c
    raise ValueError(f"a prompt of {n_tokens} tokens exceeds the captioner's limit of {TEXT_CAPACITIES[-1]} prompt tokens "
                     "(bos and eos included)")


_BUCKETS = tuple(sorted({min(max(int(x), 1), 128) for x in os.environ.get("OMNI_CAPTION_BUCKETS", "8,16,32,64,96,128").split(",")} | {128}))
CLIP_MEAN = (0.485, 0.456, 0.406)
CLIP_STD = (0.229, 0.224, 0.225)


def _legacy_to_native(sd: Dict[str, torch.Tensor]) -> Dict[str, torch.Tensor]:
    out = {}
    for k, v in sd.items():
        nk = k
        if nk.startswith("vision_tower."):
            nk = nk.replace(".proj.", ".conv.") if ".convs." in nk else nk
            nk = nk.replace(".fn.dw.", ".")
            nk = nk.replace(".window_attn.norm.", ".norm1.").replace(".channel_attn.norm.", ".norm1.")
            nk = nk.replace(".window_attn.fn.", ".window_attn.").replace(".channel_attn.fn.", ".channel_attn.")
            nk = nk.replace(".ffn.norm.", ".norm2.").replace(".ffn.fn.net.", ".ffn.")
            nk = "model." + nk
        elif nk == "image_projection":
            nk, v = "model.multi_modal_projector.image_projection.weight", v.t().contiguous()
        elif nk.startswith("image_proj_norm."):
            nk = "model.multi_modal_projector." + nk
        elif nk.startswith("image_pos_embed."):
            nk = "model.multi_modal_projector.image_position_embed." + nk[len("image_pos_embed."):]
        elif nk.startswith("visual_temporal_embed."):
            nk = "model.multi_modal_projector." + nk
        elif nk.startswith("language_model.model."):
            nk = "model.language_model." + nk[len("language_model.model."):]
        elif nk == "language_model.lm_head.weight":
            nk = "lm_head.weight"
        elif nk == "language_model.final_logits_bias":
            nk = "final_logits_bias"
        out[nk] = v
    return out


def normalise_config(cfg: dict) -> dict:
    cfg = json.loads(json.dumps(cfg))
    vc = cfg.get("vision_config")
    tc = cfg.get("text_config")
    if not isinstance(vc, dict) or not isinstance(tc, dict):
        raise ValueError("Florence-2 config.json needs `vision_config` and `text_config` objects")
# ... 828 lines not shown
                p.capture(cap.stream)
            cap.stream.synchronize()


class _DecodePlans(_StepPlans):

    def __init__(self, cap: "Florence2Captioner", B: int, R: int, max_new: int, beam=None, n_txt=None, scores=False, vocab=False):
        w, dev, dt = cap.w, cap.device, cap.dtype
        self.B, self.R = B, R
        S = (R // 32) ** 2 + 1 + (len(PROMPT_IDS) if n_txt is None else n_txt)
        self.S = S
        self.n_txt = n_txt
        pk = PlanBuilder(dev, dt)
        self.nkeys = None
        if n_txt is not None:
            self.nkeys = pk.raw((B,), torch.int32)
            self.nkeys.fill_(S)
        self.cross_kv = [pk.alloc(B, S, 1, 2 * w.d_model, zero=True) for _ in range(w.dec_layers)]
        self._keep = pk.keep
        self._build_step(cap, B, max_new, S, self.cross_kv, beam=beam, nkeys=self.nkeys, scores=scores, vocab=vocab)
        self.free_evt = None
        self._warm_up_and_capture(cap, self.step_plan)


class _CaptionPlans(_StepPlans):

    def __init__(self, cap: "Florence2Captioner", B: int, R: int, max_new: int, arena: Optional["_CaptionPlans"] = None, stream=None,
                 beam=None, n_txt=None, scores=False, force=None, controls=False, vocab=False, embed=False):
        w, dev, dt = cap.w, cap.device, cap.dtype
        if arena is not None:
            n_txt = arena.n_txt
        self.embed = bool(embed)
        self.n_txt = n_txt
        sd = w.sd
        self.B, self.R, self.T = B, R, max_new + 1
        pb = PlanBuilder(dev, dt)
        pb.reuse = bool(cap.reuse_activations)
        if arena is not None:
            assert arena.R == R and arena.B >= B and arena.arena is None
            pb.arena = iter(arena.pb.alloc_log)
        self.arena = arena
        self._row_plans = {}
        self.pb = pb
        V = pb.V
        W = _Weights(cap, pb)

        use_dma = dt == L.F32 and pb.split and os.environ.get("OMNI_GEMM_DMA", "1") != "0"
        self.use_dma = use_dma
        grp = {"dma": use_dma}

        def tokens(v: View) -> View:
            return View(v.t.view(v.B, v.H * v.W, 1, v.ld), v.coff, v.C, v.fmt)

        def linear(key, x: View, out: View, act=L.ACT_NONE, res=None, bias=True, keys=None, out_split=False):
            keys = keys or [key]
            n_out, k_in = out.C, x.C
            dma = grp["dma"] and n_out % 128 == 0 and k_in % 32 == 0 and x.ld % 16 == 0 and x.coff % 16 == 0
            assert dma or x.fmt != "split", f"{keys}: split input for a layer that cannot take the LDS-DMA GEMM"
            wp, bp = W.linear(keys, bias, dma)
            if dma and x.fmt != "split":
                pb.split_convert(x)
            xt, ot = tokens(x), tokens(out)
            pb.conv(xt, wp, bp, ot, 1, act=act, res=tokens(res) if res is not None else None, out_split=dma and out_split)
            out.fmt = ot.fmt
            return out

        def layernorm(key, x: View, out: View, add=None, period=0, eps=1e-5, split=None):
            rows = x.B * x.H * x.W
            omode, y2 = 0, None
            if grp["dma"] and split is not None and x.C % 16 == 0:
                omode, y2 = (1, None) if split is out else (2, split)
            pb.add_op(W.layernorm(key, x.ptr, out.ptr, rows, x.C, add=add.data_ptr() if add is not None else None,
                                  y2=y2.ptr if y2 is not None else None, period=period, omode=omode, eps=eps))
            out.fmt = "split" if omode == 1 else "f32"
            if y2 is not None:
                y2.fmt = "split"
            return out

        def dwconv(key, x: View, out: View):
            wp, bp = W.dwconv(key)
            pb.keep += [wp, bp]
            pb.add_op(L.make_op(L.OP_DWCONV3, dt, p=[x.ptr, wp.data_ptr(), bp.data_ptr(), None, out.ptr],
                                i={0: x.B, 1: x.H, 2: x.W, 3: x.C}))
            return out

        fuse_env = cap.fuse_dwln
        attn_split = use_dma and cap.attn_split_out

        def dwconv_ln(conv_key, norm_key, x: View, y1: View, hout: View):
            if not (fuse_env and dt == L.F32 and x.C in (128, 256, 512)):
                dwconv(conv_key, x, y1)
                return layernorm(norm_key, y1, hout, split=hout)
            wp, bp = W.dwconv(conv_key)
            pb.keep += [wp, bp]
            pb.add_op(L.make_op(L.OP_DWCONV3_LN, dt,
                                p=[x.ptr, wp.data_ptr(), bp.data_ptr(), hout.ptr, y1.ptr,
                                   W.f32(norm_key + ".weight").data_ptr(), W.f32(norm_key + ".bias").data_ptr()],
                                i={0: x.B, 1: x.H, 2: x.W, 3: x.C, 6: 1 if grp["dma"] else 0}, f={0: 1e-5}))
            hout.fmt = "split" if grp["dma"] else "f32"
            return hout

        self.x_in = pb.alloc(B, R, R, V, zero=True)
        x = self.x_in
        vt = "model.vision_tower."
        self.chan_ws = None
        self.fold_stages = []
        self.stage_out = []
        for s in range(4):
            C = w.embed_dim[s]
            grp["dma"] = use_dma and C % 128 == 0
            k, st, pd = w.patch[s]
            Ho = (x.H + 2 * pd - k) // st + 1
            conv_key = f"{vt}convs.{s}.conv"
            if w.prenorm[s]:
                xn = pb.alloc(B, x.H, x.W, x.C)
                layernorm(f"{vt}convs.{s}.norm", x, xn)
                cur = pb.alloc(B, Ho, Ho, C)
                wp, bp = W.packed(conv_key, lambda: (sd[conv_key + ".weight"], sd[conv_key + ".bias"]))
                pb.conv(xn, wp, bp, cur, k, st, pd)
                pb.release(xn, *([] if x is self.x_in else [x]))
            else:
                t0 = pb.alloc(B, Ho, Ho, C)
                if cap.patch_rows and dt == L.F32 and pb.split and V == 4 and k <= 8 and x is self.x_in:
                    wp, bp = W.cached((conv_key, dt, "patch"), lambda: (pb.pack_weight_patch(sd[conv_key + ".weight"], V),
                                                                         pb.upload(sd[conv_key + ".bias"].float())))
                    pb.conv_patch(x, wp, bp, t0, k, st, pd)
                else:
                    wp, bp = W.cached((conv_key, dt, "pad"), lambda: (pb.pack_weight(sd[conv_key + ".weight"], cin_pad=V),
                                                                       pb.upload(sd[conv_key + ".bias"].float())))
                    pb.conv(x, wp, bp, t0, k, st, pd)
                cur = pb.alloc(B, Ho, Ho, C)
                layernorm(f"{vt}convs.{s}.norm", t0, cur)
                pb.release(t0)
            H = Ho
            N = H * H
            A_, B_ = cur, pb.alloc(B, H, H, C)
            hbuf = pb.alloc(B, H, H, C)
            qkv = pb.alloc(B, H, H, 3 * C)
            att = pb.alloc(B, H, H, C)
            mlp_one = grp["dma"] and cap.fuse_mlp and C == 128 and sd[f"{vt}blocks.{s}.0.spatial_block.ffn.fc1.weight"].shape[0] == 512
            ffn = None if mlp_one else pb.alloc(B, H, H, 4 * C)
            fold = bool(cap.fold_chan_proj) and grp["dma"] and dt == L.F32 and C % 128 == 0 and N % 256 == 0 and N >= 4 * C
            chunk_tokens = 1024
            partial_tokens = 256 if fold else 0
            chunks = (N + (partial_tokens or chunk_tokens) - 1) // (partial_tokens or chunk_tokens)
            cws = pb.raw((B * w.groups[s] * chunks * 1024,), torch.float32, zero=False)
            scores_in_gemm = fold and bool(cap.chan_scores_in_gemm)
            fold_v = fold and bool(cap.fold_chan_v) and N >= 4 * C
            fold_wf = fold_wb = fold_sc = fold_mx = fold_bias = None
            if fold:
                fold_wf = pb.raw((B * C * C + (B * C if fold_v else 0),), torch.float32, zero=False)
                fold_bias = fold_wf[B * C * C:] if fold_v else None
                fold_wb = pb.raw((B * C * C,), torch.float32, zero=False)
                fold_sc = pb.raw((B,), torch.float32, zero=False)
                fold_mx = pb.raw((B * (C // 64) * w.groups[s],), torch.float32, zero=False)
            if fold:
                self.fold_stages.append(s)
            for blk in range(w.depths[s]):
                for kind in ("spatial_block", "channel_block"):
                    pre = f"{vt}blocks.{s}.{blk}.{kind}."
                    dwconv_ln(pre + "conv1", pre + "norm1", A_, B_, hbuf)
                    if kind == "spatial_block":
                        linear(pre + "window_attn.qkv", hbuf, qkv)
                        qb = W.f32(pre + "window_attn.qkv.bias")
                        nw = ((H + 11) // 12) ** 2
                        pb.add_op(L.make_op(
                            L.OP_ATTN_ROWS, dt,
                            p=[qkv.ptr, qkv.ptr, qkv.ptr, None, att.ptr, qb.data_ptr() + 4 * C, qb.data_ptr() + 8 * C],
                            i={0: 3 * C, 1: 3 * C, 2: 3 * C, 3: C, 4: 0, 5: C, 6: 2 * C, 7: 0, 8: w.heads[s], 9: 144, 10: 144,
                               11: B * nw, 12: 1, 13: H, 14: H, 15: C // w.heads[s], 16: 1 if (attn_split and grp["dma"]) else 0},
                            f={0: (C // w.heads[s]) ** -0.5}))
                        att.fmt = "split" if (attn_split and grp["dma"]) else "f32"
                        linear(pre + "window_attn.proj", att, B_, res=B_)
                    elif fold:
                        key = pre + "channel_attn.qkv"
                        wp, _ = W.linear([key], dma=True)
                        wqk, bqk, wv, bv = W.cached((key, dt, "dma-qk|v"), lambda: (
                            pb.weight_rows(wp, 0, 2 * C), pb.upload(sd[key + ".bias"][:2 * C].float()),
                            pb.weight_rows(wp, 2 * C, C), pb.upload(sd[key + ".bias"][2 * C:].float())))
                        assert hbuf.fmt == "split"
                        if scores_in_gemm:
                            wqs, bqs = W.cached((key, dt, "dma-qk-groups"), lambda: (
                                pb.pack_weight_qk_groups(wqk), pb.upload(sd[key + ".bias"][:2 * C].float()[pb.qk_group_rows(C)])))
                            pb.conv_scores(tokens(hbuf), wqs, bqs, cws, N)
                        else:
                            pb.conv(tokens(hbuf), wqk, bqk, tokens(qkv.slice(0, 2 * C)), 1)
# ... 80 lines not shown
                self.encode_plan.run(cap.stream)
                cap.stream.synchronize()
                self.encode_plan.capture(cap.stream)
                cap.stream.synchronize()
            return
        lm = "model.language_model."
        S = n_img + (len(PROMPT_IDS) if n_txt is None else n_txt)
        self.S = S
        self.prompt_ids = self.nkeys = None
        if n_txt is None:
            txt = W.cached(("prompt", dt), lambda: pb.upload((sd[lm + "shared.weight"][torch.tensor(PROMPT_IDS)] * w.embed_scale).to(torch_dtype(dt))))
            pb.keep.append(txt)
            enc = pb.alloc(B, S, 1, D)
            pb.add_op(L.make_op(L.OP_ASSEMBLE, dt, p=[img_feat.ptr, txt.data_ptr(), None, None, enc.ptr],
                                i={0: B, 1: n_img, 2: len(PROMPT_IDS), 3: D}))
        else:
            table, _ = W.token_tables()
            pb.keep.append(table)
            self.prompt_ids = pb.raw((B, n_txt), torch.int32)
            self.nkeys = pb.raw((B,), torch.int32)
            if arena is None:
                self.prompt_ids.fill_(w.pad)
                self.nkeys.fill_(S)
            enc = pb.alloc(B, S, 1, D)
            pb.add_op(L.make_op(L.OP_ASSEMBLE, dt, p=[img_feat.ptr, None, self.prompt_ids.data_ptr(), table.data_ptr(), enc.ptr],
                                i={0: B, 1: n_img, 2: n_txt, 3: D, 4: table.shape[0]}, f={0: w.embed_scale}))
        encpos = W.cached(("encpos", S, dt), lambda: pb.upload(sd[lm + "encoder.embed_positions.weight"][2:2 + S].to(torch_dtype(dt))))
        pb.keep.append(encpos)
        xa = pb.alloc(B, S, 1, D)
        dma_enc = grp["dma"] = use_dma and D % 128 == 0
        xs = pb.alloc(B, S, 1, D) if dma_enc else None
        layernorm(lm + "encoder.layernorm_embedding", enc, xa, add=encpos, period=S, split=xs)
        xin = xs if dma_enc else xa
        qkv = pb.alloc(B, S, 1, 3 * D)
        att = pb.alloc(B, S, 1, D)
        tmp = pb.alloc(B, S, 1, D)
        ffn = pb.alloc(B, S, 1, sd[lm + "encoder.layers.0.fc1.weight"].shape[0])
        nh = w.n_heads
        for l in range(w.enc_layers):
            pre = f"{lm}encoder.layers.{l}."
            linear(None, xin, qkv, keys=[pre + "self_attn.q_proj", pre + "self_attn.k_proj", pre + "self_attn.v_proj"])
            pb.add_op(L.make_op(L.OP_ATTN_ROWS, dt, p=[qkv.ptr, qkv.ptr, qkv.ptr, None, att.ptr]
                                + ([None, None, self.nkeys.data_ptr()] if self.nkeys is not None else []),
                                i={0: 3 * D, 1: 3 * D, 2: 3 * D, 3: D, 4: 0, 5: D, 6: 2 * D, 7: 0, 8: nh, 9: S, 10: S, 11: B,
                                   12: 0, 15: 64, 16: 1 if (attn_split and dma_enc) else 0}, f={0: 64 ** -0.5}))
            att.fmt = "split" if (attn_split and dma_enc) else "f32"
            linear(pre + "self_attn.out_proj", att, tmp, res=xa)
            layernorm(pre + "self_attn_layer_norm", tmp, xa, split=xs)
            linear(pre + "fc1", xin, ffn, act=L.ACT_GELU, out_split=True)
            linear(pre + "fc2", ffn, tmp, res=xa)
            layernorm(pre + "final_layer_norm", tmp, xa, split=xs)
        self.enc_out = xa
        self.cross_kv = []
        for l in range(w.dec_layers):
            pre = f"{lm}decoder.layers.{l}.encoder_attn."
            kv = pb.alloc(B, S, 1, 2 * D)
            linear(None, xin, kv, keys=[pre + "k_proj", pre + "v_proj"])
            self.cross_kv.append(kv)
        self.free_evt = None
        self.n_encode_ops = len(pb.ops)
        self.encode_flops = pb.flops
        self.encode_plan = pb.build()
        if arena is not None:
            assert len(pb.alloc_log) == len(arena.pb.alloc_log) and self.n_encode_ops == arena.n_encode_ops, \
                "arena replay: the two builds made different allocation / op sequences"
            if cap.use_graph:
                self.encode_plan.capture(stream or cap.stream)
            return
        self._build_step(cap, B, max_new, S, self.cross_kv, pb.ws, beam=beam, nkeys=self.nkeys, scores=scores, force=force, controls=controls,
                         vocab=vocab)
        self._warm_up_and_capture(cap, self.encode_plan, self.step_plan)

    def set_prompt(self, ids: torch.Tensor, nkeys: torch.Tensor, n: int):
        assert self.prompt_ids is not None and ids.shape[-1] == self.n_txt and n <= self.B
        self.prompt_ids[:n].copy_(ids.expand(n, -1), non_blocking=True)
        self.nkeys[:n].copy_(nkeys.expand(n), non_blocking=True)

    def rows_for(self, cap: "Florence2Captioner", n: int) -> int:
        last, cap._last_remainder = getattr(cap, "_last_remainder", None), n
        if n in self._row_plans or n == last:
            return n
        return min(cap.bucket(n), self.B)

    def encode_rows(self, cap: "Florence2Captioner", n: int, stream=None) -> "_CaptionPlans":
        assert self.arena is None and 1 <= n <= self.B
        if n == self.B:
            return self
        cp = self._row_plans.pop(n, None)
        if cp is None:
            while len(self._row_plans) >= max(1, int(cap.row_graphs)):
                if dev_sync := (cap.device.type == "cuda"):
                    torch.cuda.synchronize(cap.device)
                self._row_plans.pop(next(iter(self._row_plans)))
            cp = _CaptionPlans(cap, n, self.R, self.T - 1, arena=self, stream=stream)
            cap.row_graph_builds = getattr(cap, "row_graph_builds", 0) + 1
        self._row_plans[n] = cp
        return cp


class _Config(SimpleNamespace):
    pass


class Florence2Captioner:
    fuse_dwln = True
    attn_split_out = True
    fold_chan_proj = True
    fold_chan_v = True
    chan_scores_in_gemm = True
    fuse_mlp = True
    exact_rows = os.environ.get("OMNI_EXACT_ROWS", "1") != "0"
    row_graphs = int(os.environ.get("OMNI_CAPTION_ROW_GRAPHS", "24"))
    patch_rows = os.environ.get("OMNI_PATCH_ROWS", "1") != "0"
    reuse_activations = True

    long_kv_budget_bytes = 2 ** 30

    def __init__(self, model_dir, device=None, precision: Optional[str] = None, resolution: Optional[int] = None):
        device = L.require_device(device, "Florence2Captioner")
        L.lib()
        self.device = device
        precision = precision or os.environ.get("OMNI_PRECISION", "f32")
        self.dtype = L.F32 if precision == "f32" else L.F16
        self.resolution = int(resolution or os.environ.get("OMNI_CAPTION_RES", "768"))
        self.w = FlorenceWeights(model_dir)
        self.config = _Config(name_or_path=str(model_dir) if "florence" in str(model_dir).lower() else f"florence:{model_dir}",
                              model_type="florence2")
        self.use_graph = os.environ.get("OMNI_HIPGRAPH", "1") != "0"
        self.stream = self._lane_stream(0)
        self._wcache = {}
        self._plans = {}
        self.max_new_tokens = 20
        self.early_exit_every = 5
        self.num_beams = 1
        self.token_scores = False
        self.last_steps = 0
        self._lut, self._bic = None, {}
        self._lock = L.DeviceLock(self.device, reentrant=True)

    def to(self, *a, **k):
        return self

    def eval(self):
        return self

    @staticmethod
    def bucket(n: int) -> int:
        for b in _BUCKETS:
            if n <= b:
                return b
        return _BUCKETS[-1]

    def max_new_limit(self) -> int:
        return int(self.w.sd["model.language_model.decoder.embed_positions.weight"].shape[0]) - 2

    def check_max_new(self, max_new_tokens, beam=None) -> int:
        lim, why = self.max_new_limit(), "the decoder's position table has no row beyond that"
        if beam and beam_max_new(beam[0]) < lim:
            lim, why = beam_max_new(beam[0]), f"beam search with num_beams={beam[0]} stages every position of its beams in LDS"
        n = max_new_tokens
        if isinstance(n, bool) or not isinstance(n, int) or n < 1 or n > lim:
            raise ValueError(f"max_new_tokens must be an integer in 1..{lim} ({why}), got {n!r}")
        return n
# ... 139 lines not shown
        w = self.w
        return CaptionVocabulary.of(vocabulary).check(w.vocab, max_new_tokens, w.eos, w.forced_bos, w.forced_eos, w.ngram, w.start)

    def prompt_batch(self, rows, R):
        rows = [[int(t) for t in r] for r in rows]
        if all(r == PROMPT_IDS for r in rows):
            return None
        vocab = self.w.sd["model.language_model.shared.weight"].shape[0]
        for r in rows:
            if not r:
                raise ValueError("an empty prompt: at least one token is needed")
            bad = [t for t in r if not 0 <= t < vocab]
            if bad:
                raise ValueError(f"prompt token id {bad[0]} is outside the token table (0..{vocab - 1})")
        n_txt = text_capacity(max(len(r) for r in rows))
        n_img = (R // 32) ** 2 + 1
        ids = torch.full((len(rows), n_txt), int(self.w.pad), dtype=torch.int32)
        for b, r in enumerate(rows):
            ids[b, :len(r)] = torch.tensor(r, dtype=torch.int32)
        nkeys = torch.tensor([n_img + len(r) for r in rows], dtype=torch.int32)
        return ids, nkeys, n_txt

    def _prompt_from_input_ids(self, input_ids, attention_mask, n, R):
        if input_ids is None:
            if attention_mask is not None:
                raise ValueError("attention_mask without input_ids")
            return None
        ids = torch.as_tensor(input_ids).detach().cpu().long()
        n_img = (R // 32) ** 2 + 1
        img_tok = int(self.w.cfg.get("image_token_id", 51289))
        if ids.dim() != 2 or ids.shape[0] != n:
            raise ValueError(f"input_ids must be [batch, tokens] with one row per image ({n}), got {tuple(ids.shape)}")
        if ids.shape[1] <= n_img or not bool((ids[:, :n_img] == img_tok).all()):
            raise ValueError(f"input_ids must start with the {n_img} image placeholder tokens (id {img_tok}) of a {R}x{R} image, "
                             "followed by the prompt")
        txt = ids[:, n_img:]
        if attention_mask is None:
            lens = [txt.shape[1]] * n
        else:
            m = torch.as_tensor(attention_mask).detach().cpu()
            if tuple(m.shape) != tuple(ids.shape):
                raise ValueError(f"attention_mask {tuple(m.shape)} does not match input_ids {tuple(ids.shape)}")
            m = m != 0
            if not bool(m[:, :n_img].all()):
                raise ValueError("attention_mask hides image tokens: only prompt padding can be masked")
            mt = m[:, n_img:]
            lens = mt.sum(1).tolist()
            if not bool((mt == (torch.arange(txt.shape[1])[None, :] < mt.sum(1)[:, None])).all()):
                raise ValueError("attention_mask must be right-padded (ones, then zeros): left padding and holes are not supported")
        return self.prompt_batch([txt[b, :lens[b]].tolist() for b in range(n)], R)

    def _encode_into(self, cp: _CaptionPlans, n: int, dec: _DecodePlans, row0: int, stream=None):
        stream = stream or self.stream
        assert cp.n_txt == dec.n_txt, "the micro-batches and their merged decode plan have one text capacity"
        if dec.nkeys is not None:
            dec.nkeys[row0:row0 + n].copy_(cp.nkeys[:n], non_blocking=True)
        if n < cp.B and self.exact_rows:
            cp = cp.encode_rows(self, cp.rows_for(self, n), stream)
        (cp.encode_plan.replay if self.use_graph else cp.encode_plan.run)(stream)
        for src, dst in zip(cp.cross_kv, dec.cross_kv):
            dst.t[row0:row0 + n].copy_(src.t[:n], non_blocking=True)

    def _decode_merged(self, dec: _DecodePlans, n: int, max_new: int, stream=None) -> torch.Tensor:
        stream = stream or self.stream
        run = dec.step_plan.replay if self.use_graph else dec.step_plan.run
        for _ in range(max_new):
            run(stream)
        self.last_steps = max_new
        return dec.snapshot(n)

    def _lane_stream(self, k):
        return torch.cuda.Stream(device=self.device)

    @property
    def stream2(self):
        if getattr(self, "_stream2", None) is None:
            self._stream2 = self._lane_stream(1)
        return self._stream2

    def encode_lane(self, k):
        if k == 0:
            return self.stream
        if k == 1:
            return self.stream2
        extra = self.__dict__.setdefault("_extra_lanes", {})
        if k not in extra:
            extra[k] = self._lane_stream(k)
        return extra[k]

    @property
    def dec_stream(self):
        if getattr(self, "_dec_stream", None) is None:
            self._dec_stream = self._lane_stream(2)
        return self._dec_stream

    def _run(self, cp: _CaptionPlans, n: int, max_new: int, defer: bool = False, embeds: Optional[list] = None, after=None) -> torch.Tensor:
        run = (lambda p: p.replay(self.stream)) if self.use_graph else (lambda p: p.run(self.stream))
        run(cp.encode_plan)
        if embeds is not None:
            embeds.append(self._embed_rows(cp, n))
        poll = 0 if defer else self.early_exit_every
        steps = 0
        for t in range(max_new):
            run(cp.step_plan)
            steps += 1
            if poll and (t + 1) % poll == 0 and t + 1 < max_new and bool(cp.finished[:n].min().item()):
                break
        self.last_steps = steps
        if after is not None:
            return after(cp, n)
        if defer:
            return cp.snapshot(n)
# ... 373 lines not shown
```

omniparser_amd/pipeline.py:

```python
import contextlib
import os
from types import SimpleNamespace
from typing import List, Optional, Sequence

import numpy as np
import torch

from . import _lib as L
from .florence import Florence2Captioner, caption_confidence
from .util import utils as U
from .util.yolov9 import YOLOv9Detector


OCR_CAP = 1024
MASK_WORDS = OCR_CAP // 64


def _f64_bits(x: float):
    import struct
    lo, hi = struct.unpack("<ii", struct.pack("<d", float(x)))
    return lo, hi


class _GlueState:
# ... 223 lines not shown
        return U.rank_elements(frame, elements, {"model": self.cap, "processor": self.proc}, queries, top_k=top_k)

    def embed(self, frame: torch.Tensor, elements):
        return U.embed_elements(frame, elements, {"model": self.cap, "processor": self.proc})

    def match(self, frame: torch.Tensor, elements, exemplars, top_k=5):
        return U.match_elements(frame, elements, {"model": self.cap, "processor": self.proc}, exemplars, top_k=top_k)

    def track(self, prev_frame: torch.Tensor, prev_elements, frame: torch.Tensor, elements, min_score=0.9):
        return U.track_elements(self.embed(prev_frame, prev_elements), self.embed(frame, elements), min_score=min_score)

    def prompt_ids(self, prompt):
        if prompt is None:
            return None
        if isinstance(prompt, str):
            return self.proc.prompt_ids(prompt)
        return [int(t) for t in prompt]

    @torch.inference_mode()
    def caption_launch(self, frames: Sequence[torch.Tensor], crops_per_frame, max_new_tokens=None, crops_dev: Optional[torch.Tensor] = None,
                       overlap=False, prompt=None, scores=False):
        cap = self.cap
        R = cap.resolution
        prompt = self.prompt_ids(prompt)
        pr = cap.prompt_batch([prompt], R) if prompt is not None else None
        pkw = {}
        if pr is not None:
            pkw = {"n_txt": pr[2]}
            held = self.__dict__.setdefault("_prompt_dev", {})
            if (tuple(prompt), R) not in held:
                if len(held) >= 8:
                    torch.cuda.synchronize(cap.device)
                    held.clear()
                held[(tuple(prompt), R)] = (pr[0].to(cap.device), pr[1].to(cap.device))
            pr_ids, pr_keys = held[(tuple(prompt), R)]
        max_new_tokens = max_new_tokens or self.max_new_tokens
        if crops_dev is not None:
            flat = [(fi, k) for fi, n in enumerate(crops_per_frame) for k in range(int(n))]
        else:
            flat = [(fi, b) for fi, cl in enumerate(crops_per_frame) for b in cl]
        ids_all = []
        merged = len(flat) > self.batch_size and os.environ.get("OMNI_MERGED_DECODE", "1") != "0"
        beam = cap.beam_config()
        lanes = [cap.encode_lane(k) for k in range(max(1, self.encode_lanes))] if overlap else [cap.stream]
        cap.begin_batch()
        if overlap and merged:
            self._dec_slot = 1 - getattr(self, "_dec_slot", 1)
        bkw = {"beam": beam} if beam else {}
        if scores or getattr(cap, "token_scores", False):
            if beam:
                raise ValueError("caption confidence needs greedy decoding (num_beams = 1): beam search has no token scores")
            bkw = {"scores": True}
        dec = cap.decode_plans(cap.decode_bucket(len(flat)), R, max_new_tokens, slot=self._dec_slot if overlap else 0, **bkw, **pkw) if merged else None
        if merged and not overlap:
            with torch.cuda.stream(cap.stream):
                dec.reset()
        if not overlap:
            self._ev["cap0"] = cap.stream.record_event(torch.cuda.Event(enable_timing=True))
        used = []
        for mbi, s in enumerate(range(0, len(flat), self.batch_size)):
            chunk = flat[s:s + self.batch_size]
            n = len(chunk)
            lane = 0
            if overlap and merged:
                lane = self._mb_count = (getattr(self, "_mb_count", -1) + 1) % len(lanes)
            stream = lanes[lane]
            if merged and cap.exact_rows and n < self.batch_size:
                cp = cap.plans(cap.bucket(self.batch_size), R, max_new_tokens, slot=lane, **pkw)
            else:
                cp = cap.plans(cap.bucket(n), R, max_new_tokens, slot=lane if n == self.batch_size else 0, **({} if merged else bkw), **pkw)
            with torch.cuda.stream(stream):
                if cp.free_evt is not None:
                    stream.wait_event(cp.free_evt)
                if merged and dec.free_evt is not None and stream not in used:
                    stream.wait_event(dec.free_evt)
                if not merged:
                    cp.reset()
                c64, tmp = cap.crop_scratch(n, R)
                if crops_dev is None:
                    bx = torch.tensor([b for _, b in chunk], dtype=torch.int32).to(cap.device, non_blocking=True)
                o = 0
                while o < n:
                    fi = chunk[o][0]
                    e = o
                    while e < n and chunk[e][0] == fi:
                        e += 1
                    rects = crops_dev[fi, chunk[o][1]:] if crops_dev is not None else bx[o:]
                    cap.launch_crops(cp, o, e - o, frames[fi], rects, c64[o:], tmp[o:] if tmp is not None else None, stream)
                    o = e
                if pr is not None:
                    cp.set_prompt(pr_ids, pr_keys, n)
                if merged:
                    cap._encode_into(cp, n, dec, s, stream)
                else:
                    ids_all.append(cap._run(cp, n, max_new_tokens, defer=True))
                if overlap:
                    cp.free_evt = stream.record_event()
            if stream not in used:
                used.append(stream)
        ids_stream = cap.stream
        if merged and not overlap:
            with torch.cuda.stream(cap.stream):
                self._ev["cap1"] = cap.stream.record_event(torch.cuda.Event(enable_timing=True))
                ids_all.append(cap._decode_merged(dec, len(flat), max_new_tokens))
                self._ev["cap2"] = cap.stream.record_event(torch.cuda.Event(enable_timing=True))
        elif merged:
# ... 313 lines not shown
```

omniparser_amd/planner.py:

```python
import math
import os
from dataclasses import dataclass
from typing import Optional

import torch

from . import _lib as L


def vec_width(dtype: int) -> int:
    return 4 if dtype == L.F32 else 8


def torch_dtype(dtype: int):
    return torch.float32 if dtype == L.F32 else torch.float16


@dataclass
class View:
    t: torch.Tensor
    coff: int
    C: int
    fmt: str = "f32"

    @property
    def B(self): return self.t.shape[0]
    @property
    def H(self): return self.t.shape[1]
    @property
    def W(self): return self.t.shape[2]
    @property
    def ld(self): return self.t.shape[3]
    @property
    def ptr(self): return self.t.data_ptr()

    def slice(self, off, c):
        assert 0 <= off and off + c <= self.C, (off, c, self.C)
        return View(self.t, self.coff + off, c, self.fmt)

    def torch(self):
        return self.t[..., self.coff:self.coff + self.C].permute(0, 3, 1, 2).float()


import weakref

_TENSORS = {}


def _register(t: torch.Tensor, role: str) -> torch.Tensor:
    if not t.numel():
        return t
    nbytes = t.numel() * t.element_size()
    ent = _TENSORS.get(t.data_ptr())
    if ent is not None:
        old = ent[0]()
        if old is not None and old.data_ptr() == t.data_ptr() and ent[2] >= nbytes and old is not t:
            return t
    if len(_TENSORS) > 4096 and len(_TENSORS) % 1024 == 0:
        live_tensors()
    _TENSORS[t.data_ptr()] = (weakref.ref(t), role, nbytes)
    return t


def live_tensors():
    out = []
    for ptr, (ref, role, nbytes) in list(_TENSORS.items()):
        t = ref()
        if t is None or t.data_ptr() != ptr:
            _TENSORS.pop(ptr, None)
            continue
        out.append((ptr, nbytes, role, t))
    return sorted(out, key=lambda r: r[0])


def conv_key(M, N, K, k, s) -> str:
    return f"{M}x{N}x{K}k{k}s{s}"


class PlanBuilder:
    workspace_on_host = False

    def __init__(self, device, dtype: int):
        self.device = torch.device(device)
        self.dtype = dtype
        self.V = vec_width(dtype)
        self.ops = []
        self.keep = []
        self.split = os.environ.get("OMNI_CONV_SPLIT", "1") == "1"
        self.ws = None
        self.ws_kib = 32 * 1024
        self.cnt = None
        self.n_cnt = 4096 if os.environ.get("OMNI_SPLITK_COMBINE", "0") == "1" else 0
        self.conv_tuning = None
        self.reuse = False
        self._free, self._released, self._pins = [], set(), []
        self.reused_bytes = 0
        self.alloc_log = []
        self.arena = None
        self.flops = 0
        self.bytes = 0

    def alloc(self, B, H, W, C, zero=False) -> View:
        tdt = torch_dtype(self.dtype)
        if self.arena is not None:
            return View(self._from_arena((B, H, W, C), tdt), 0, C)
        if not zero:
            t = self._from_free((B, H, W, C), tdt)
            if t is not None:
                self.alloc_log.append(t)
                return View(t, 0, C)
        fn = torch.zeros if zero else torch.empty
        t = fn((B, H, W, C), dtype=tdt, device=self.device)
        self.keep.append(_register(t, "zero" if zero else "scratch"))
        self.alloc_log.append(t)
        return View(t, 0, C)

    def raw(self, shape, dtype, zero=True) -> torch.Tensor:
        if self.arena is not None:
            return self._from_arena(tuple(shape), dtype)
        if not zero:
            t = self._from_free(tuple(shape), dtype)
            if t is not None:
                self.alloc_log.append(t)
                return t
        t = (torch.zeros if zero else torch.empty)(shape, dtype=dtype, device=self.device)
        self.keep.append(_register(t, "zero" if zero else "scratch"))
        self.alloc_log.append(t)
        return t

# ... 42 lines not shown
        self.keep.append(_register(t, "const"))
        return t

    @staticmethod
    def split_f16(w2d: torch.Tensor) -> torch.Tensor:
        cout, K = w2d.shape
        assert K % 16 == 0
        w2d = w2d.float().clamp(-65504.0, 65504.0)
        hi = w2d.to(torch.float16)
        lo = ((w2d - hi.float()) * 2048.0).to(torch.float16)
        return torch.cat([hi.view(cout, K // 16, 16), lo.view(cout, K // 16, 16)], -1).contiguous()

    @staticmethod
    def split_f16_b(w2d: torch.Tensor):
        cout, K = w2d.shape
        assert K % 16 == 0
        w2d = w2d.double()
        amax = float(w2d.abs().max())
        k = 0 if amax == 0.0 else 12 - math.floor(math.log2(amax))
        k = max(-24, min(24, k))
        ws = (w2d * (2.0 ** k)).float()
        hi = ws.to(torch.float16)
        lo = (ws - hi.float()).to(torch.float16)
        return torch.cat([hi.view(cout, K // 16, 16), lo.view(cout, K // 16, 16)], -1).contiguous(), 2.0 ** -k

    KPERM16 = (0, 1, 2, 3, 8, 9, 10, 11, 4, 5, 6, 7, 12, 13, 14, 15)

    def pack_weight_dma(self, w: torch.Tensor, kperm: bool = False) -> torch.Tensor:
        w2d = w.detach().float().reshape(w.shape[0], -1)
        if kperm:
            cout, K = w2d.shape
            assert K % 16 == 0
            w2d = w2d.view(cout, K // 16, 16)[:, :, list(self.KPERM16)].reshape(cout, K).contiguous()
        t, oscale = self.split_f16_b(w2d)
        t = self.upload(t)
        t.omni_fmt, t.omni_oscale = 2, oscale
        return t

    def pack_weight(self, w: torch.Tensor, cin_pad: Optional[int] = None) -> torch.Tensor:
        w = w.detach().float()
        cout, cin, kh, kw = w.shape
        if cin_pad and cin_pad > cin:
            w = torch.cat([w, w.new_zeros(cout, cin_pad - cin, kh, kw)], 1)
        w = w.permute(0, 2, 3, 1).reshape(cout, -1)
        cin_eff = max(cin, cin_pad or 0)
        if self.split and self.dtype == L.F32 and cin_eff % 32 == 0 and cin_eff * kh * kw >= 128:
            t = self.upload(self.split_f16(w))
            t.omni_fmt = 1
            return t
        return self.upload(w.to(torch_dtype(self.dtype)))

    def conv(self, x: View, w_packed: torch.Tensor, bias: Optional[torch.Tensor], out: View, k: int, s: int = 1,
             p: Optional[int] = None, act: int = L.ACT_NONE, res: Optional[View] = None, scale: float = 0.0,
             out_split: bool = False):
        p = k // 2 if p is None else p
        Ho = (x.H + 2 * p - k) // s + 1
        Wo = (x.W + 2 * p - k) // s + 1
        assert (out.B, out.H, out.W) == (x.B, Ho, Wo), ((out.B, out.H, out.W), (x.B, Ho, Wo))
        cout = out.C
        wfmt = getattr(w_packed, "omni_fmt", 0) if self.dtype == L.F32 else 0
        if wfmt:
            assert w_packed.dtype == torch.float16 and w_packed.numel() == 2 * cout * k * k * x.C and x.C % 32 == 0, \
                (tuple(w_packed.shape), cout, k, x.C)
        else:
            assert tuple(w_packed.shape) == (cout, k * k * x.C), (tuple(w_packed.shape), cout, k, x.C)
        if wfmt == 2:
            assert k == 1 and s == 1 and p == 0 and scale == 0.0 and cout % 128 == 0, "format-B weights: pointwise layers, Cout % 128 == 0"
            assert x.fmt == "split", "the LDS-DMA GEMM reads a pre-split input: its producer must emit format B (or insert split_convert)"
            assert x.ld % 16 == 0 and x.coff % 16 == 0 and not (out_split and (res is not None or out.ld % 16 or out.coff % 16))
        else:
            assert x.fmt == "f32" and not out_split, "register-staged conv kernels read and write f32"
        if res is not None:
            assert (res.B, res.H, res.W, res.C) == (out.B, out.H, out.W, out.C) and res.fmt == "f32"
        b = None
        if bias is not None:
            b = bias if bias.device == self.device and bias.dtype == torch.float32 else self.upload(bias.detach().float())
            ent = _TENSORS.get(b.data_ptr())
            if ent is None or ent[0]() is not b:
                _register(b, "const")
            self.keep.append(b)
            assert b.numel() == cout
        if self.ws is None and (self.device.type == "cuda" or self.workspace_on_host):
            self.ws = self.raw((self.ws_kib * 256,), torch.float32, zero=False)
        if self.cnt is None and self.ws is not None and self.n_cnt and wfmt == 1:
            self.cnt = self.raw((self.n_cnt,), torch.int32, zero=True)
        cnt = self.cnt if (wfmt == 1 and self.cnt is not None) else None
        tune = (0, 0)
        if wfmt == 1 and self.conv_tuning:
            tune = tuple(self.conv_tuning.get(conv_key(x.B * Ho * Wo, cout, k * k * x.C, k, s), (0, 0)))
        op = L.make_op(
            L.OP_CONV, self.dtype,
            p=[x.ptr, w_packed.data_ptr(), b.data_ptr() if b is not None else None,
               res.ptr if res is not None else None, out.ptr, self.ws.data_ptr() if self.ws is not None else None,
               cnt.data_ptr() if cnt is not None else None],
            i={0: x.B, 1: x.H, 2: x.W, 3: x.C, 4: x.ld, 5: x.coff, 6: k, 7: k, 8: s, 9: p, 10: Ho, 11: Wo,
               12: cout, 13: out.ld, 14: out.coff, 15: act,
               16: res.ld if res is not None else 0, 17: res.coff if res is not None else 0,
               19: self.ws_kib if self.ws is not None else 0, 20: wfmt, 21: 1 if out_split else 0,
               22: tune[0], 23: tune[1], 24: cnt.numel() if cnt is not None else 0},
            f={0: scale, 1: getattr(w_packed, "omni_oscale", 0.0) if wfmt == 2 else 0.0})
        self.ops.append(op)
        self.keep.append(w_packed)
        out.fmt = "split" if out_split else "f32"
        M = x.B * Ho * Wo
        esz = 4 if self.dtype == L.F32 else 2
        self.flops += 2 * M * cout * k * k * x.C
        self.bytes += esz * (x.B * x.H * x.W * x.C + w_packed.numel() // (2 if wfmt else 1) + M * cout * (2 if res is not None else 1))
        return out

    @staticmethod
    def weight_rows(w_packed: torch.Tensor, row0: int, rows: int) -> torch.Tensor:
        assert getattr(w_packed, "omni_fmt", 0) == 2 and 0 <= row0 and row0 + rows <= w_packed.shape[0]
        t = w_packed[row0:row0 + rows]
        t.omni_fmt, t.omni_oscale = 2, w_packed.omni_oscale
        return t

    def conv_per_image(self, x: View, w_img: torch.Tensor, scales: torch.Tensor, bias: Optional[torch.Tensor], out: View,
                       res: Optional[View], rows_per_img: int, bias_per_image: bool = False):
        cout, K = out.C, x.C
        M = x.B * x.H * x.W
        assert self.dtype == L.F32 and x.fmt == "split" and x.ld % 16 == 0 and x.coff % 16 == 0 and cout % 128 == 0 and K % 32 == 0
        assert (out.B, out.H, out.W) == (x.B, x.H, x.W) and M % rows_per_img == 0
        nimg = M // rows_per_img
        assert w_img.numel() * w_img.element_size() >= nimg * cout * K * 4 and scales.dtype == torch.float32 and scales.numel() >= nimg
        if bias_per_image:
            assert bias is not None and bias.dtype == torch.float32 and bias.numel() >= nimg * cout and bias.device.type == self.device.type
        else:
            assert bias is None or (bias.dtype == torch.float32 and bias.numel() == cout and bias.device.type == self.device.type)
        if res is not None:
            assert (res.B, res.H, res.W, res.C) == (out.B, out.H, out.W, out.C) and res.fmt == "f32"
        self.ops.append(L.make_op(
            L.OP_CONV, self.dtype,
            p=[x.ptr, w_img.data_ptr(), bias.data_ptr() if bias is not None else None, res.ptr if res is not None else None, out.ptr,
               None, scales.data_ptr()],
            i={0: x.B, 1: x.H, 2: x.W, 3: K, 4: x.ld, 5: x.coff, 6: 1, 7: 1, 8: 1, 9: 0, 10: x.H, 11: x.W, 12: cout, 13: out.ld, 14: out.coff,
               15: L.ACT_NONE, 16: res.ld if res is not None else 0, 17: res.coff if res is not None else 0, 20: 2,
               26: rows_per_img, 27: cout * K * 4, **({29: 1} if bias_per_image else {})}))
        self.keep += [w_img, scales] + ([bias] if bias is not None else [])
        out.fmt = "f32"
        self.flops += 2 * M * cout * K
        self.bytes += 4 * (M * K + nimg * cout * K + M * cout * (2 if res is not None else 1))
        return out

    def fold_gemm(self, w_img: torch.Tensor, scales: torch.Tensor, wvt: torch.Tensor, out: torch.Tensor, nimg: int, C: int):
        assert self.dtype == L.F32 and C % 128 == 0 and getattr(wvt, "omni_fmt", 0) == 2 and wvt.numel() == 2 * C * C
        assert w_img.numel() * w_img.element_size() >= nimg * C * C * 4 and out.numel() >= nimg * C * C and out.dtype == torch.float32
        assert scales.dtype == torch.float32 and scales.numel() >= nimg
        self.ops.append(L.make_op(
            L.OP_CONV, self.dtype,
            p=[w_img.data_ptr(), wvt.data_ptr(), None, None, out.data_ptr(), None, scales.data_ptr()],
            i={0: nimg, 1: C, 2: 1, 3: C, 4: C, 5: 0, 6: 1, 7: 1, 8: 1, 9: 0, 10: C, 11: 1, 12: C, 13: C, 14: 0, 15: L.ACT_NONE, 20: 2,
               26: C, 27: 0}))
        self.keep += [w_img, scales, wvt, out]

    def repack_per_image(self, wf: torch.Tensor, w_img: torch.Tensor, scales: torch.Tensor, maxima: torch.Tensor, nimg: int, C: int):
        assert self.dtype == L.F32 and C % 64 == 0 and wf.numel() >= nimg * C * C and w_img.numel() * w_img.element_size() >= nimg * C * C * 4
        assert scales.numel() >= nimg and maxima.numel() >= nimg * (C // 64) * (C // 32)
        self.ops.append(L.make_op(L.OP_SPLIT_CONVERT, self.dtype,
                                  p=[wf.data_ptr(), None, None, None, w_img.data_ptr(), maxima.data_ptr(), scales.data_ptr()],
                                  i={0: nimg, 1: C, 3: C, 4: C, 5: 0, 6: 1, 13: C, 14: 0}))
        self.keep += [wf, w_img, scales, maxima]

    @staticmethod
    def qk_group_rows(C: int):
        assert C % 32 == 0
        return [part * C + g * 32 + r for g in range(C // 32) for part in (0, 1) for r in range(32)]

    def pack_weight_qk_groups(self, w_qk: torch.Tensor) -> torch.Tensor:
        assert getattr(w_qk, "omni_fmt", 0) == 2 and w_qk.shape[0] % 64 == 0
        idx = torch.tensor(self.qk_group_rows(w_qk.shape[0] // 2), device=w_qk.device)
        t = self.upload(w_qk[idx])
        t.omni_fmt, t.omni_oscale = 2, w_qk.omni_oscale
        return t

    def conv_scores(self, x: View, w_qk: torch.Tensor, bias: Optional[torch.Tensor], ws: torch.Tensor, rows_per_img: int):
        cout, K = w_qk.shape[0], x.C
        M = x.B * x.H * x.W
        assert self.dtype == L.F32 and x.fmt == "split" and x.ld % 16 == 0 and x.coff % 16 == 0 and K % 32 == 0
        assert getattr(w_qk, "omni_fmt", 0) == 2 and w_qk.numel() == 2 * cout * K and cout % 256 == 0
        assert rows_per_img > 0 and rows_per_img % 256 == 0 and M % rows_per_img == 0
        assert ws.dtype == torch.float32 and ws.numel() >= (M // 256) * (cout // 64) * 1024
        assert bias is None or (bias.dtype == torch.float32 and bias.numel() == cout and bias.device.type == self.device.type)
        self.ops.append(L.make_op(
            L.OP_CONV, self.dtype,
            p=[x.ptr, w_qk.data_ptr(), bias.data_ptr() if bias is not None else None, None, None, None, None, ws.data_ptr()],
            i={0: x.B, 1: x.H, 2: x.W, 3: K, 4: x.ld, 5: x.coff, 6: 1, 7: 1, 8: 1, 9: 0, 10: x.H, 11: x.W, 12: cout, 13: cout, 14: 0,
               15: L.ACT_NONE, 20: 2, 26: rows_per_img, 27: 0, 28: 1},
            f={1: w_qk.omni_oscale}))
        self.keep += [w_qk, ws] + ([bias] if bias is not None else [])
        self.flops += 2 * M * cout * K + 2 * M * cout * 16
        self.bytes += 4 * (M * K + cout * K + (M // 256) * (cout // 64) * 1024)

    def pack_weight_patch(self, w: torch.Tensor, ld: int = 4) -> torch.Tensor:
        w = w.detach().float()
        cout, cin, kh, kw = w.shape
        assert kh == kw and kh <= 8 and cin <= ld == 4
        full = w.new_zeros(cout, kh, 8, ld)
        full[:, :, :kw, :cin] = w.permute(0, 2, 3, 1)
        t = self.upload(self.split_f16(full.reshape(cout, kh * 8 * ld)))
        t.omni_fmt = 1
        return t

    def conv_patch(self, x: View, w_patch: torch.Tensor, bias: torch.Tensor, out: View, k: int, s: int, p: int, act: int = L.ACT_NONE):
        assert self.dtype == L.F32 and x.fmt == "f32" and x.ld == 4 and x.coff == 0 and x.C == 4 and k <= 8
        Ho = (x.H + 2 * p - k) // s + 1
        Wo = (x.W + 2 * p - k) // s + 1
        cout = out.C
        assert (out.B, out.H, out.W) == (x.B, Ho, Wo) and w_patch.numel() == 2 * cout * k * 32 and getattr(w_patch, "omni_fmt", 0) == 1
        assert bias.device.type == self.device.type and bias.dtype == torch.float32 and bias.numel() == cout
        if self.ws is None and (self.device.type == "cuda" or self.workspace_on_host):
            self.ws = self.raw((self.ws_kib * 256,), torch.float32, zero=False)
        self.ops.append(L.make_op(
            L.OP_CONV, self.dtype,
            p=[x.ptr, w_patch.data_ptr(), bias.data_ptr(), None, out.ptr, self.ws.data_ptr() if self.ws is not None else None],
            i={0: x.B, 1: x.H, 2: x.W, 3: 32, 4: 4, 5: 0, 6: k, 7: 1, 8: s, 9: p, 10: Ho, 11: Wo, 12: cout, 13: out.ld, 14: out.coff,
               15: act, 19: self.ws_kib if self.ws is not None else 0, 20: 1, 25: 1}))
        self.keep += [w_patch, bias]
        out.fmt = "f32"
        M = x.B * Ho * Wo
        self.flops += 2 * M * cout * k * k * x.C
        self.bytes += 4 * (x.B * x.H * x.W * x.C + cout * k * k * x.C + M * cout)
        return out

    def mlp_fused(self, x: View, w1: torch.Tensor, b1: torch.Tensor, w2: torch.Tensor, b2: torch.Tensor, res: View, out: View):
        C, hid = x.C, b1.numel()
        assert self.dtype == L.F32 and x.fmt == "split" and res.fmt == "f32" and (C, hid) == (128, 512), (x.fmt, res.fmt, C, hid)
        assert getattr(w1, "omni_fmt", 0) == 2 and getattr(w2, "omni_fmt", 0) == 2 and w1.numel() == 2 * hid * C == w2.numel()
        assert (out.B, out.H, out.W, out.C) == (x.B, x.H, x.W, C) == (res.B, res.H, res.W, res.C) and b2.numel() == C
        rows = x.B * x.H * x.W
        self.ops.append(L.make_op(L.OP_MLP_FUSED, self.dtype,
                                  p=[x.ptr, w1.data_ptr(), b1.data_ptr(), res.ptr, out.ptr, w2.data_ptr(), b2.data_ptr()],
                                  i={0: rows, 1: 1, 3: C, 4: x.ld, 5: x.coff, 12: hid, 13: out.ld, 14: out.coff, 16: res.ld, 17: res.coff},
                                  f={1: w1.omni_oscale, 2: w2.omni_oscale}))
        self.keep += [w1, w2, b1, b2]
        out.fmt = "f32"
        self.flops += 2 * rows * C * hid * 2
        self.bytes += 4 * (rows * C * 3 + 2 * C * hid)
        return out

    def split_convert(self, x: View, out: Optional[View] = None) -> View:
        out = out or x
        assert self.dtype == L.F32 and x.fmt == "f32" and x.C % 16 == 0 and (out.B, out.H, out.W, out.C) == (x.B, x.H, x.W, x.C)
        self.ops.append(L.make_op(L.OP_SPLIT_CONVERT, self.dtype, p=[x.ptr, None, None, None, out.ptr],
                                  i={0: x.B * x.H * x.W, 1: 1, 3: x.C, 4: x.ld, 5: x.coff, 13: out.ld, 14: out.coff}))
        self.bytes += 8 * x.B * x.H * x.W * x.C
        out.fmt = "split"
        return out

    def _pool(self, kind, x: View, out: View, k=0, s=1, p=0, accumulate=0):
        assert x.C == out.C and x.B == out.B
        op = L.make_op(
            kind, self.dtype, p=[x.ptr, None, None, None, out.ptr],
            i={0: x.B, 1: x.H, 2: x.W, 3: x.C, 4: x.ld, 5: x.coff, 6: k, 8: s, 9: p, 10: out.H, 11: out.W,
               13: out.ld, 14: out.coff, 18: accumulate})
        self.ops.append(op)
        esz = 4 if self.dtype == L.F32 else 2
        self.bytes += esz * (x.B * x.H * x.W * x.C + out.B * out.H * out.W * out.C * (2 if accumulate else 1))
        return out

    def avgpool2(self, x: View, out: View):
        assert (out.H, out.W) == (x.H - 1, x.W - 1)
        return self._pool(L.OP_AVGPOOL2, x, out)

    def maxpool(self, x: View, out: View, k, s, p):
        assert (out.H, out.W) == ((x.H + 2 * p - k) // s + 1, (x.W + 2 * p - k) // s + 1)
        return self._pool(L.OP_MAXPOOL, x, out, k, s, p)

    def resize_nearest(self, x: View, out: View, accumulate=False):
        return self._pool(L.OP_RESIZE_NEAREST, x, out, accumulate=1 if accumulate else 0)

    def resize_sum(self, srcs, out: View):
        assert 1 <= len(srcs) <= 5 and all(s.C == out.C and s.B == out.B for s in srcs)
        if len(srcs) == 1:
            return self.resize_nearest(srcs[0], out)
        x = srcs[0]
# ... 20 lines not shown
```

Before: 13.48.

## Fuse stem LayerNorm into patch conv and write cross-attn KV directly into decode buffers

Adds a LayerNorm epilogue to the split-f16 conv kernel so the captioner stem conv normalizes its 128-channel output tile in LDS, removing a separate LayerNorm pass. It also adds an indirect output base: the KV projection GEMMs read their output pointer from a device word that a new SET_BASES op rewrites before each encode replay. Encoded cross-attention K/V then land directly in the merged decode buffers instead of being copied afterwards. The cost is extra pointer-table launches, more validation, and an LDS-staged epilogue that only applies to unsplit 128x128 tiles.

New measurement: 13.59 (median of 6 runs). No clear change (+0.8%).

```diff
diff --git a/include/omni_amd.h b/include/omni_amd.h
--- a/include/omni_amd.h
+++ b/include/omni_amd.h
@@ -65,6 +65,12 @@
   OMNI_OP_REGION_OCR = OMNI_OP_VISUAL_MATCH + 1,
   OMNI_OP__END
 };
+
+enum {
+  OMNI_OP_SET_BASES = OMNI_OP_REGION_OCR + 1
+};
+
+#define OMNI_SET_BASES_MAX 8
 
 #define OMNI_OCR_CLASS_STRIP 1000
 #define OMNI_OCR_CLASS_TEXT 1001
diff --git a/omniparser_amd/_lib.py b/omniparser_amd/_lib.py
--- a/omniparser_amd/_lib.py
+++ b/omniparser_amd/_lib.py
@@ -14,6 +14,8 @@
 OP_GREEDY_VOCAB_STEP = 27
 OP_VISUAL_MATCH = 28
 OP_REGION_OCR = 29
+OP_SET_BASES = 30
+SET_BASES_MAX = 8
 OCR_CLASS_STRIP, OCR_CLASS_TEXT, OCR_CLASS_HARD = 1000, 1001, 1002
 CAND_BYTES = 32
 ABI_VERSION = 3
diff --git a/omniparser_amd/bundle.py b/omniparser_amd/bundle.py
--- a/omniparser_amd/bundle.py
+++ b/omniparser_amd/bundle.py
@@ -164,4 +164,4 @@
     for j in range(3):
         ints[f"mean{j}"] = f32_bits(CLIP_MEAN[j])
         ints[f"std{j}"] = f32_bits(CLIP_STD[j])
-    return write_bundle(path, {"encode": cp.encode_plan.ops, "step": cp.step_plan.ops}, named, ints)
+    return write_bundle(path, {"encode": planner.direct_ops(cp.encode_plan.ops), "step": cp.step_plan.ops}, named, ints)
diff --git a/omniparser_amd/csrc/capi.hip b/omniparser_amd/csrc/capi.hip
--- a/omniparser_amd/csrc/capi.hip
+++ b/omniparser_amd/csrc/capi.hip
@@ -72,6 +72,7 @@
     case OMNI_OP_GREEDY_VOCAB_STEP: return omni_launch_vocab_step(op, s);
     case OMNI_OP_VISUAL_MATCH: return omni_launch_visual_match(op, s);
     case OMNI_OP_REGION_OCR: return omni_launch_region_ocr(op, s);
+    case OMNI_OP_SET_BASES: return omni_launch_set_bases(op, s);
     default:
       omni_set_error("unknown op kind %d", op->kind);
       return OMNI_E_ARG;
@@ -110,8 +111,13 @@
         ext[7] = (M / 256) * (Cout / 64) * 4096;
         ext[4] = 1;
       }
-      break;
-    }
+      if (i[20] == 2 && i[30] == 1) ext[7] = 8;
+      if (i[20] == 1 && i[31] == 1) ext[6] = ext[7] = Cout * 4;
+      break;
+    }
+    case OMNI_OP_SET_BASES:
+      ext[4] = (long long)(i[0] > 0 ? i[0] : 1) * 8;
+      break;
     case OMNI_OP_CHAN_ATTN: {
       const long long B = i[0], N = i[1], C = i[3], G = i[4], ct = i[10] > 0 ? i[10] : (i[5] > 0 ? i[5] : 1);
       ext[0] = B * N * 3 * C * esz; ext[4] = B * N * C * esz; ext[5] = B * G * ((N + ct - 1) / ct) * 1024 * 4;
@@ -258,28 +264,34 @@
   for (int k = 0; k < 8; ++k) if (ext[k] < 1) ext[k] = 1;
 }
 
+static int check_range(const omni_op_t* op, int index, const char* what, int k, const void* ptr, long long bytes) {
+  hipDeviceptr_t base = nullptr;
+  size_t size = 0;
+  hipError_t e = hipMemGetAddressRange(&base, &size, (hipDeviceptr_t)ptr);
+  if (e != hipSuccess || !base) {
+    (void)hipGetLastError();
+    omni_set_error("op %d (kind %d): %s[%d] = %p is not inside any device allocation (%s)", index, op->kind, what, k, ptr,
+                   e != hipSuccess ? hipGetErrorString(e) : "no base");
+    return OMNI_E_ARG;
+  }
+  const long long off = (const char*)ptr - (const char*)base;
+  if (off < 0 || off + bytes > (long long)size) {
+    omni_set_error("op %d (kind %d): %s[%d] = %p + %lld bytes runs past its allocation [%p, +%zu)", index, op->kind, what, k, ptr, bytes,
+                   (void*)base, size);
+    return OMNI_E_ARG;
+  }
+  return OMNI_OK;
+}
+
 static int check_op_ptrs(const omni_op_t* op, int index) {
   long long ext[8];
   op_extents(op, ext);
-  for (int k = 0; k < 8; ++k) {
-    const void* ptr = op->p[k];
-    if (!ptr) continue;
-    hipDeviceptr_t base = nullptr;
-    size_t size = 0;
-    hipError_t e = hipMemGetAddressRange(&base, &size, (hipDeviceptr_t)ptr);
-    if (e != hipSuccess || !base) {
-      (void)hipGetLastError();
-      omni_set_error("op %d (kind %d): p[%d] = %p is not inside any device allocation (%s)", index, op->kind, k, ptr,
-                     e != hipSuccess ? hipGetErrorString(e) : "no base");
-      return OMNI_E_ARG;
-    }
-    const long long off = (const char*)ptr - (const char*)base;
-    if (off < 0 || off + ext[k] > (long long)size) {
-      omni_set_error("op %d (kind %d): p[%d] = %p + %lld bytes runs past its allocation [%p, +%zu)", index, op->kind, k, ptr, ext[k],
-                     (void*)base, size);
-      return OMNI_E_ARG;
-    }
-  }
+  for (int k = 0; k < 8; ++k)
+    if (op->p[k])
+      if (int rc = check_range(op, index, "p", k, op->p[k], ext[k])) return rc;
+  if (op->kind == OMNI_OP_SET_BASES && op->i[0] >= 1 && op->i[0] <= OMNI_SET_BASES_MAX && op->i[1] > 0 && op->i[2] > 0 && op->i[3] >= 0 && op->i[4] > 0)
+    for (int k = 0; k < op->i[0]; ++k)
+      if (int rc = check_range(op, index, "target", k, (const void*)(uintptr_t)omni_set_bases_target(op, k), omni_set_bases_span(op))) return rc;
   return OMNI_OK;
 }
 
diff --git a/omniparser_amd/csrc/conv_igemm.hip b/omniparser_amd/csrc/conv_igemm.hip
--- a/omniparser_amd/csrc/conv_igemm.hip
+++ b/omniparser_amd/csrc/conv_igemm.hip
@@ -18,6 +18,7 @@
   int* cnt;
   float scale;
   int vec_px;
+  const float* ln_g; const float* ln_b; float ln_eps;
 };
 
 
@@ -343,7 +344,7 @@
   }
 }
 
-template <int BM, int BN, int NW, bool PW>
+template <int BM, int BN, int NW, bool PW, bool LN = false>
 __global__ __launch_bounds__(NW * 64, 2) void conv_split_kernel(ConvArgs a) {
   constexpr int RB = 128, ROWB = RB + 16, VPR = 8, RPP = NW * 8;
   constexpr int BKE = 32;
@@ -489,6 +490,44 @@
   }
 
   const float inv = 1.0f / 2048.0f;
+  if constexpr (LN) {
+    static_assert(BN == 128 && TN == 1 && BM % (2 * NW) == 0, "LN epilogue: one 128-channel tile per row, two rows per wave and pass");
+    constexpr int LP = BN * 4 + 16;
+    static_assert(BM * LP <= 2 * STAGE, "the staged tile must fit the LDS ring");
+    {
+      const int n = wn * (BN / WN) + (lane & 31);
+      const float bias = a.bias ? a.bias[n] : 0.0f;
+#pragma unroll
+      for (int i = 0; i < TM; ++i) {
+        const int rb = wm * (BM / 2) + i * 32 + 4 * (lane >> 5);
+#pragma unroll
+        for (int e = 0; e < 16; ++e)
+          *reinterpret_cast<float*>(lds + (rb + (e & 3) + 8 * (e >> 2)) * LP + n * 4) = (accM[i][0][e] + accC[i][0][e] * inv) + bias;
+      }
+    }
+    __syncthreads();
+    const int lr = lane & 31, sub = lane >> 5;
+    const f32x4 g = *reinterpret_cast<const f32x4*>(a.ln_g + lr * 4), b = *reinterpret_cast<const f32x4*>(a.ln_b + lr * 4);
+    auto group_sum = [](float v) {
+#pragma unroll
+      for (int o = 16; o > 0; o >>= 1) v += __shfl_xor(v, o);
+      return v;
+    };
+    float* __restrict__ Y = reinterpret_cast<float*>(a.y) + a.out_coff + lr * 4;
+#pragma unroll
+    for (int pass = 0; pass < BM / (2 * NW); ++pass) {
+      const int r = (pass * NW + wave) * 2 + sub;
+      const f32x4 t = *reinterpret_cast<const f32x4*>(lds + r * LP + lr * 16);
+      const float mean = group_sum((t[0] + t[1]) + (t[2] + t[3])) / (float)BN;
+      const f32x4 d = t - mean;
+      const float rstd = 1.0f / sqrtf(group_sum((d[0] * d[0] + d[1] * d[1]) + (d[2] * d[2] + d[3] * d[3])) / (float)BN + a.ln_eps);
+      float o[4];
+#pragma unroll
+      for (int e = 0; e < 4; ++e) o[e] = (t[e] - mean) * rstd * g[e] + b[e];
+      if (m0 + r < a.M) *reinterpret_cast<f32x4*>(Y + (long long)(m0 + r) * a.ldo) = f32x4{o[0], o[1], o[2], o[3]};
+    }
+    return;
+  }
   if (a.splits > 1) {
     float* __restrict__ P = a.ws + (long long)blockIdx.z * a.M * a.Cout;
     const bool combine = a.cnt != nullptr;
@@ -572,7 +611,8 @@
   dim3 grid(tile_grid(a.mtiles, a.ntiles, a.xcd_order, a.xcd_n), 1, a.splits);
   const bool pw = p.loader == CONV_LOADER_POINTWISE;
   if constexpr (BM == 128 && BN == 128) {
-    if (pw) hipLaunchKernelGGL((conv_split_kernel<BM, BN, 8, true>), grid, dim3(512), 0, s, a);
+    if (a.ln_g) hipLaunchKernelGGL((conv_split_kernel<BM, BN, 8, false, true>), grid, dim3(512), 0, s, a);
+    else if (pw) hipLaunchKernelGGL((conv_split_kernel<BM, BN, 8, true>), grid, dim3(512), 0, s, a);
     else hipLaunchKernelGGL((conv_split_kernel<BM, BN, 8, false>), grid, dim3(512), 0, s, a);
   } else {
     if (pw) hipLaunchKernelGGL((conv_split_kernel<BM, BN, 4, true>), grid, dim3(256), 0, s, a);
@@ -720,8 +760,22 @@
   if (op->i[20]) {
     OMNI_REQUIRE(op->dtype == OMNI_F32 && a.Cin % 32 == 0, "conv: split-f16 mode needs f32 activations and Cin %% 32 == 0");
     OMNI_REQUIRE(op->i[24] >= 0 && (op->i[24] == 0 || op->p[6]), "conv: i24 arrival counters without p6");
-    return plan_split(a, ws_bytes, op->i[22], op->i[23], op->i[24] > 0 ? (int*)op->p[6] : nullptr, op->i[24], p);
-  }
+    OMNI_REQUIRE(op->i[31] == 0 || op->i[31] == 1, "conv: unknown epilogue mode %d (i31)", op->i[31]);
+    if (int rc = plan_split(a, ws_bytes, op->i[22], op->i[23], op->i[24] > 0 ? (int*)op->p[6] : nullptr, op->i[24], p)) return rc;
+    if (op->i[31] == 1) {
+      OMNI_REQUIRE(p.bm == 128 && p.bn == 128 && a.Cout == 128,
+                   "conv: the LayerNorm epilogue (i31) needs the 128x128 tile to cover Cout (tile %dx%d, Cout %d)", p.bm, p.bn, a.Cout);
+      OMNI_REQUIRE(a.splits == 1, "conv: the LayerNorm epilogue (i31) takes no split-K (%d splits)", a.splits);
+      OMNI_REQUIRE(a.act == OMNI_ACT_NONE, "conv: the LayerNorm epilogue (i31) takes no activation (act %d)", a.act);
+      OMNI_REQUIRE(!a.res && a.scale == 0.0f && op->i[24] == 0, "conv: the LayerNorm epilogue (i31) takes no residual, output scale or arrival counters");
+      OMNI_REQUIRE(p.loader != CONV_LOADER_POINTWISE, "conv: the LayerNorm epilogue (i31) is built for the aligned / row-patch loader");
+      OMNI_REQUIRE(op->p[6] && op->p[7] && (uintptr_t)op->p[6] % 16 == 0 && (uintptr_t)op->p[7] % 16 == 0 && a.ldo % 4 == 0 && a.out_coff % 4 == 0 &&
+                   (uintptr_t)a.y % 16 == 0, "conv: the LayerNorm epilogue (i31) needs gamma (p6) and beta (p7), 16-byte aligned like y / ldo / out_coff");
+      a.ln_g = (const float*)op->p[6]; a.ln_b = (const float*)op->p[7]; a.ln_eps = op->f[2];
+    }
+    return OMNI_OK;
+  }
+  OMNI_REQUIRE(op->i[31] == 0, "conv: the LayerNorm epilogue (i31) needs split-f16 mode (i20 = 1)");
   return plan_typed(a, V, ws_bytes, op->i[22], p);
 }
 
diff --git a/omniparser_amd/csrc/gemm_dma.hip b/omniparser_amd/csrc/gemm_dma.hip
--- a/omniparser_amd/csrc/gemm_dma.hip
+++ b/omniparser_amd/csrc/gemm_dma.hip
@@ -20,6 +20,7 @@
 };
 
 constexpr int GEMM_EPI_SCORES = 3;
+constexpr int GEMM_EPI_IND = 4;
 
 #if defined(__AMDGCN__)
 struct RowBuf {
@@ -37,9 +38,18 @@
 };
 #endif
 
+__device__ __forceinline__ unsigned char* load_base_word(const unsigned char* word) {
+#if defined(__AMDGCN__)
+  typedef const __attribute__((address_space(4))) unsigned long long* cword_t;
+  return reinterpret_cast<unsigned char*>((uintptr_t)*(cword_t)(uintptr_t)word);
+#else
+  return reinterpret_cast<unsigned char*>((uintptr_t)*reinterpret_cast<const unsigned long long*>(word));
+#endif
+}
+
 template <int BM, int BN, int WM, int WN, int TM, int TN, int LDS_BYTES, int ACT, bool OSPLIT, bool RES>
-__device__ __forceinline__ void gemm_epilogue(f32x16 (&acc)[TM][TN], const GemmArgs& a, const float* bias, unsigned char* lds, int m0, int n0, int wave,
-                                              int lane, float osc) {
+__device__ __forceinline__ void gemm_epilogue(f32x16 (&acc)[TM][TN], const GemmArgs& a, unsigned char* y, const float* bias, unsigned char* lds, int m0,
+                                              int n0, int wave, int lane, float osc) {
   constexpr int NW = WM * WN;
   const int wm = wave / WN, wn = wave % WN;
   const int hsel = lane >> 5;
@@ -51,8 +61,8 @@
   float amax = 0.0f;
   const int rrow = lane >> 4, chunk = lane & 15;
   const int trows = min(a.M - m0, BM), wc0 = n0 + wn * (BN / WN);
-  const RowBuf ybuf(a.y + ((long long)m0 * a.ldo + a.out_coff + wc0) * 4, (unsigned)(trows - 1) * (unsigned)(a.ldo * 4) + (BN / WN) * 4);
-  const RowBuf rbuf(RES ? reinterpret_cast<const unsigned char*>(a.res) + ((long long)m0 * a.ldr + a.res_coff + wc0) * 4 : a.y,
+  const RowBuf ybuf(y + ((long long)m0 * a.ldo + a.out_coff + wc0) * 4, (unsigned)(trows - 1) * (unsigned)(a.ldo * 4) + (BN / WN) * 4);
+  const RowBuf rbuf(RES ? reinterpret_cast<const unsigned char*>(a.res) + ((long long)m0 * a.ldr + a.res_coff + wc0) * 4 : y,
                     RES ? (unsigned)(trows - 1) * (unsigned)(a.ldr * 4) + (BN / WN) * 4 : 0u);
   const unsigned yoff = (unsigned)(wm * (BM / WM) + rrow) * (unsigned)(a.ldo * 4) + chunk * 16;
   const unsigned roff = (unsigned)(wm * (BM / WM) + rrow) * (unsigned)(a.ldr * 4) + chunk * 16;
@@ -392,9 +402,13 @@
 
   if constexpr (ACT == GEMM_EPI_SCORES)
     gemm_scores_epilogue<BM, BN, WM, WN, TM, TN, NSTAGE * STAGE>(acc, a, lds, img, __builtin_amdgcn_readfirstlane(mt) - img * a.img_tiles, n0, wave, lane, osc);
+  else if constexpr (ACT == GEMM_EPI_IND)
+    gemm_epilogue<BM, BN, WM, WN, TM, TN, NSTAGE * STAGE, OMNI_ACT_NONE, OSPLIT, RES>(acc, a, load_base_word(a.y),
+                                                                                      a.bias + (long long)img * a.bias_img_stride, lds, m0, n0,
+                                                                                      wave, lane, osc);
   else
-    gemm_epilogue<BM, BN, WM, WN, TM, TN, NSTAGE * STAGE, ACT, OSPLIT, RES>(acc, a, a.bias + (long long)img * a.bias_img_stride, lds, m0, n0, wave,
-                                                                            lane, osc);
+    gemm_epilogue<BM, BN, WM, WN, TM, TN, NSTAGE * STAGE, ACT, OSPLIT, RES>(acc, a, a.y, a.bias + (long long)img * a.bias_img_stride, lds, m0, n0,
+                                                                            wave, lane, osc);
 #endif
 }
 
@@ -552,12 +566,12 @@
       }
   }
   omni_report_range(amax);
-  gemm_epilogue<NW * 32, C, NW, 1, 1, OB, 2 * STAGE, OMNI_ACT_NONE, false, true>(acc2, a.ep, a.ep.bias, lds, m0, 0, wave, lane, a.ep.oscale);
+  gemm_epilogue<NW * 32, C, NW, 1, 1, OB, 2 * STAGE, OMNI_ACT_NONE, false, true>(acc2, a.ep, a.ep.y, a.ep.bias, lds, m0, 0, wave, lane, a.ep.oscale);
 #endif
 }
 
 template <int BM, int BN, int WM, int WN, int NSTAGE>
-int launch_tile(GemmArgs& a, int rows_per_img, int act, int osplit, bool scores, hipStream_t s) {
+int launch_tile(GemmArgs& a, int rows_per_img, int act, int osplit, bool scores, bool ind, hipStream_t s) {
   if (rows_per_img % BM != 0) {
     omni_set_error("gemm_dma: per-image weights need whole %d-row tiles per image (rows per image %d)", BM, rows_per_img);
     return OMNI_E_ARG;
@@ -579,7 +593,8 @@
     }                                                                                                                              \
     hipLaunchKernelGGL((gemm_dma_kernel<BM, BN, WM, WN, NSTAGE, ACT_, OS_, RES_, SCHED1>), grid, block, 0, s, a);                  \
   } while (0)
-  if (scores) {
+  if (ind) OMNI_GD(GEMM_EPI_IND, false, false);
+  else if (scores) {
     if constexpr (BM == 256 && BN == 256) OMNI_GD(GEMM_EPI_SCORES, false, false);
     else { omni_set_error("gemm_dma: the scores epilogue is built for the 256x256 tile"); return OMNI_E_ARG; }
   }
@@ -659,11 +674,53 @@
     else if (!strcmp(e, "256x256") && a.N % 256 == 0) tile = 0;
   }
   if (scores) tile = 0;
+  OMNI_REQUIRE(op->i[30] == 0 || op->i[30] == 1, "gemm_dma: unknown output-base mode %d (i30)", op->i[30]);
+  const bool ind = op->i[30] == 1;
+  if (ind) {
+    OMNI_REQUIRE(!scores && act == OMNI_ACT_NONE && !osplit && !a.res,
+                 "gemm_dma: an indirect output base (i30) takes no scores epilogue, activation, format-B output or residual");
+    OMNI_REQUIRE(op->p[7] && (uintptr_t)op->p[7] % 8 == 0, "gemm_dma: the output-base word (p7) must be an 8-byte aligned pointer");
+    a.y = (unsigned char*)op->p[7];
+  }
   int rc;
-  if (tile == 0) rc = launch_tile<256, 256, 2, 4, 2>(a, rows_per_img, act, osplit, scores, s);
-  else if (tile == 1) rc = launch_tile<256, 128, 4, 2, 3>(a, rows_per_img, act, osplit, false, s);
-  else rc = launch_tile<128, 128, 2, 2, 2>(a, rows_per_img, act, osplit, false, s);
+  if (tile == 0) rc = launch_tile<256, 256, 2, 4, 2>(a, rows_per_img, act, osplit, scores, ind, s);
+  else if (tile == 1) rc = launch_tile<256, 128, 4, 2, 3>(a, rows_per_img, act, osplit, false, ind, s);
+  else rc = launch_tile<128, 128, 2, 2, 2>(a, rows_per_img, act, osplit, false, ind, s);
   if (rc) return rc;
+  OMNI_HIP_CHECK(hipGetLastError());
+  return OMNI_OK;
+}
+
+namespace {
+struct BaseWords { unsigned long long* table; unsigned long long v[OMNI_SET_BASES_MAX]; int n; };
+__global__ __launch_bounds__(64) void set_bases_kernel(BaseWords a) {
+  const int k = threadIdx.x;
+  if (k < a.n) a.table[k] = a.v[k];
+}
+}
+
+unsigned long long omni_set_bases_target(const omni_op_t* op, int k) {
+  return (unsigned long long)(uint32_t)op->i[16 + 2 * k] | ((unsigned long long)(uint32_t)op->i[17 + 2 * k] << 32);
+}
+
+long long omni_set_bases_span(const omni_op_t* op) {
+  return (((long long)op->i[1] - 1) * op->i[2] + op->i[3] + op->i[4]) * 4;
+}
+
+int omni_launch_set_bases(const omni_op_t* op, hipStream_t s) {
+  const int n = op->i[0];
+  OMNI_REQUIRE(n >= 1 && n <= OMNI_SET_BASES_MAX, "set_bases: %d words (i0; 1..%d)", n, OMNI_SET_BASES_MAX);
+  OMNI_REQUIRE(op->p[4] && (uintptr_t)op->p[4] % 8 == 0, "set_bases: the table (p4) must be an 8-byte aligned pointer");
+  OMNI_REQUIRE(op->i[1] > 0 && op->i[2] > 0 && op->i[3] >= 0 && op->i[4] > 0 && op->i[3] + op->i[4] <= op->i[2],
+               "set_bases: bad target extent (rows %d, ld %d, channel offset %d, channels %d)", op->i[1], op->i[2], op->i[3], op->i[4]);
+  BaseWords a{};
+  a.table = (unsigned long long*)op->p[4];
+  a.n = n;
+  for (int k = 0; k < n; ++k) {
+    a.v[k] = omni_set_bases_target(op, k);
+    OMNI_REQUIRE(a.v[k] != 0 && a.v[k] % 16 == 0, "set_bases: target %d = %p is not a 16-byte aligned address", k, (void*)(uintptr_t)a.v[k]);
+  }
+  hipLaunchKernelGGL(set_bases_kernel, dim3(1), dim3(64), 0, s, a);
   OMNI_HIP_CHECK(hipGetLastError());
   return OMNI_OK;
 }
diff --git a/omniparser_amd/csrc/omni_internal.h b/omniparser_amd/csrc/omni_internal.h
--- a/omniparser_amd/csrc/omni_internal.h
+++ b/omniparser_amd/csrc/omni_internal.h
@@ -166,6 +166,9 @@
 
 int omni_launch_conv(const omni_op_t* op, hipStream_t s);
 int omni_launch_gemm_dma(const omni_op_t* op, hipStream_t s);
+int omni_launch_set_bases(const omni_op_t* op, hipStream_t s);
+unsigned long long omni_set_bases_target(const omni_op_t* op, int k);
+long long omni_set_bases_span(const omni_op_t* op);
 int omni_launch_split_convert(const omni_op_t* op, hipStream_t s);
 int omni_launch_chan_repack(const omni_op_t* op, hipStream_t s);
 int omni_launch_mlp_fused(const omni_op_t* op, hipStream_t s);
diff --git a/omniparser_amd/florence.py b/omniparser_amd/florence.py
--- a/omniparser_amd/florence.py
+++ b/omniparser_amd/florence.py
@@ -10,7 +10,7 @@
 import torch
 
 from . import _lib as L
-from .planner import PlanBuilder, View, torch_dtype
+from .planner import PlanBuilder, View, set_bases_op, torch_dtype
 
 PROMPT_IDS = [0, 2264, 473, 5, 2274, 6190, 116, 2]
 TEXT_CAPACITIES = (8, 16, 32, 64)
@@ -945,7 +945,7 @@
         def tokens(v: View) -> View:
             return View(v.t.view(v.B, v.H * v.W, 1, v.ld), v.coff, v.C, v.fmt)
 
-        def linear(key, x: View, out: View, act=L.ACT_NONE, res=None, bias=True, keys=None, out_split=False):
+        def linear(key, x: View, out: View, act=L.ACT_NONE, res=None, bias=True, keys=None, out_split=False, base_word=None):
             keys = keys or [key]
             n_out, k_in = out.C, x.C
             dma = grp["dma"] and n_out % 128 == 0 and k_in % 32 == 0 and x.ld % 16 == 0 and x.coff % 16 == 0
@@ -954,7 +954,8 @@
             if dma and x.fmt != "split":
                 pb.split_convert(x)
             xt, ot = tokens(x), tokens(out)
-            pb.conv(xt, wp, bp, ot, 1, act=act, res=tokens(res) if res is not None else None, out_split=dma and out_split)
+            pb.conv(xt, wp, bp, ot, 1, act=act, res=tokens(res) if res is not None else None, out_split=dma and out_split,
+                    base_word=base_word if dma else None)
             out.fmt = ot.fmt
             return out
 
@@ -998,6 +999,7 @@
         vt = "model.vision_tower."
         self.chan_ws = None
         self.fold_stages = []
+        self.stem_ln_fused = False
         self.stage_out = []
         for s in range(4):
             C = w.embed_dim[s]
@@ -1013,18 +1015,29 @@
                 pb.conv(xn, wp, bp, cur, k, st, pd)
                 pb.release(xn, *([] if x is self.x_in else [x]))
             else:
-                t0 = pb.alloc(B, Ho, Ho, C)
-                if cap.patch_rows and dt == L.F32 and pb.split and V == 4 and k <= 8 and x is self.x_in:
+                patch = cap.patch_rows and dt == L.F32 and pb.split and V == 4 and k <= 8 and x is self.x_in
+                if patch:
                     wp, bp = W.cached((conv_key, dt, "patch"), lambda: (pb.pack_weight_patch(sd[conv_key + ".weight"], V),
                                                                          pb.upload(sd[conv_key + ".bias"].float())))
-                    pb.conv_patch(x, wp, bp, t0, k, st, pd)
+                if arena is not None:
+                    self.stem_ln_fused = arena.stem_ln_fused
                 else:
-                    wp, bp = W.cached((conv_key, dt, "pad"), lambda: (pb.pack_weight(sd[conv_key + ".weight"], cin_pad=V),
-                                                                       pb.upload(sd[conv_key + ".bias"].float())))
-                    pb.conv(x, wp, bp, t0, k, st, pd)
-                cur = pb.alloc(B, Ho, Ho, C)
-                layernorm(f"{vt}convs.{s}.norm", t0, cur)
-                pb.release(t0)
+                    self.stem_ln_fused = bool(patch and cap.fuse_stem_ln and C == 128 and pb.patch_fuses_ln(x, C, k, st, pd))
+                if self.stem_ln_fused:
+                    cur = pb.alloc(B, Ho, Ho, C)
+                    nk = f"{vt}convs.{s}.norm"
+                    pb.conv_patch(x, wp, bp, cur, k, st, pd, ln=(W.f32(nk + ".weight"), W.f32(nk + ".bias"), 1e-5), tile=3, splits=1)
+                else:
+                    t0 = pb.alloc(B, Ho, Ho, C)
+                    if patch:
+                        pb.conv_patch(x, wp, bp, t0, k, st, pd)
+                    else:
+                        wp, bp = W.cached((conv_key, dt, "pad"), lambda: (pb.pack_weight(sd[conv_key + ".weight"], cin_pad=V),
+                                                                           pb.upload(sd[conv_key + ".bias"].float())))
+                        pb.conv(x, wp, bp, t0, k, st, pd)
+                    cur = pb.alloc(B, Ho, Ho, C)
+                    layernorm(f"{vt}convs.{s}.norm", t0, cur)
+                    pb.release(t0)
             H = Ho
             N = H * H
             A_, B_ = cur, pb.alloc(B, H, H, C)
@@ -1211,11 +1224,20 @@
             layernorm(pre + "final_layer_norm", tmp, xa, split=xs)
         self.enc_out = xa
         self.cross_kv = []
+        self.kv_table = None
+        if (arena.kv_table is not None) if arena is not None else (bool(cap.kv_direct) and dma_enc and w.dec_layers <= L.SET_BASES_MAX):
+            self.kv_table = pb.raw((w.dec_layers,), torch.int64)
         for l in range(w.dec_layers):
             pre = f"{lm}decoder.layers.{l}.encoder_attn."
             kv = pb.alloc(B, S, 1, 2 * D)
-            linear(None, xin, kv, keys=[pre + "k_proj", pre + "v_proj"])
+            linear(None, xin, kv, keys=[pre + "k_proj", pre + "v_proj"], base_word=self.kv_table[l:l + 1] if self.kv_table is not None else None)
             self.cross_kv.append(kv)
+        self._kv_ops = {}
+        if self.kv_table is not None:
+            if arena is None:
+                self.kv_table.copy_(torch.tensor([kv.ptr for kv in self.cross_kv], dtype=torch.int64))
+            else:
+                assert [kv.ptr for kv in self.cross_kv] == [kv.ptr for kv in arena.cross_kv]
         self.free_evt = None
         self.n_encode_ops = len(pb.ops)
         self.encode_flops = pb.flops
@@ -1234,6 +1256,19 @@
         assert self.prompt_ids is not None and ids.shape[-1] == self.n_txt and n <= self.B
         self.prompt_ids[:n].copy_(ids.expand(n, -1), non_blocking=True)
         self.nkeys[:n].copy_(nkeys.expand(n), non_blocking=True)
+
+    def kv_bases_op(self, dst=None, row0: int = 0):
+        dst = dst or self.cross_kv
+        key = (tuple(d.ptr for d in dst), row0)
+        op = self._kv_ops.get(key)
+        if op is None:
+            kv = self.cross_kv[0]
+            S, row_bytes = kv.H, kv.H * kv.ld * kv.t.element_size()
+            assert all((d.H, d.ld, d.coff, d.C) == (S, kv.ld, kv.coff, kv.C) and row0 + self.B <= d.B for d in dst)
+            if len(self._kv_ops) >= 64:
+                self._kv_ops.clear()
+            op = self._kv_ops[key] = set_bases_op(self.kv_table, [d.ptr + row0 * row_bytes for d in dst], self.B * S, kv.ld, kv.coff, kv.C)
+        return op
 
     def rows_for(self, cap: "Florence2Captioner", n: int) -> int:
         last, cap._last_remainder = getattr(cap, "_last_remainder", None), n
@@ -1268,6 +1303,8 @@
     fold_chan_v = True
     chan_scores_in_gemm = True
     fuse_mlp = True
+    fuse_stem_ln = True
+    kv_direct = True
     exact_rows = os.environ.get("OMNI_EXACT_ROWS", "1") != "0"
     row_graphs = int(os.environ.get("OMNI_CAPTION_ROW_GRAPHS", "24"))
     patch_rows = os.environ.get("OMNI_PATCH_ROWS", "1") != "0"
@@ -1513,12 +1550,21 @@
 
     def _encode_into(self, cp: _CaptionPlans, n: int, dec: _DecodePlans, row0: int, stream=None):
         stream = stream or self.stream
+        last = row0 + n == getattr(dec, "n_crops", None)
         assert cp.n_txt == dec.n_txt, "the micro-batches and their merged decode plan have one text capacity"
         if dec.nkeys is not None:
             dec.nkeys[row0:row0 + n].copy_(cp.nkeys[:n], non_blocking=True)
         if n < cp.B and self.exact_rows:
             cp = cp.encode_rows(self, cp.rows_for(self, n), stream)
-        (cp.encode_plan.replay if self.use_graph else cp.encode_plan.run)(stream)
+        run = cp.encode_plan.replay if self.use_graph else cp.encode_plan.run
+        if self.kv_direct and cp.kv_table is not None and row0 + cp.B <= dec.B and (cp.B == n or last):
+            L.launch(cp.kv_bases_op(dec.cross_kv, row0), stream)
+            try:
+                run(stream)
+            finally:
+                L.launch(cp.kv_bases_op(), stream)
+            return
+        run(stream)
         for src, dst in zip(cp.cross_kv, dec.cross_kv):
             dst.t[row0:row0 + n].copy_(src.t[:n], non_blocking=True)
 
diff --git a/omniparser_amd/pipeline.py b/omniparser_amd/pipeline.py
--- a/omniparser_amd/pipeline.py
+++ b/omniparser_amd/pipeline.py
@@ -299,6 +299,8 @@
                 raise ValueError("caption confidence needs greedy decoding (num_beams = 1): beam search has no token scores")
             bkw = {"scores": True}
         dec = cap.decode_plans(cap.decode_bucket(len(flat)), R, max_new_tokens, slot=self._dec_slot if overlap else 0, **bkw, **pkw) if merged else None
+        if merged:
+            dec.n_crops = len(flat)
         if merged and not overlap:
             with torch.cuda.stream(cap.stream):
                 dec.reset()
diff --git a/omniparser_amd/planner.py b/omniparser_amd/planner.py
--- a/omniparser_amd/planner.py
+++ b/omniparser_amd/planner.py
@@ -75,6 +75,28 @@
 
 def conv_key(M, N, K, k, s) -> str:
     return f"{M}x{N}x{K}k{k}s{s}"
+
+
+def set_bases_op(table: torch.Tensor, targets, rows: int, ld: int, coff: int, cout: int) -> "L.OmniOp":
+    targets = [int(t) for t in targets]
+    assert table.dtype == torch.int64 and 1 <= len(targets) <= min(L.SET_BASES_MAX, table.numel())
+    i = {0: len(targets), 1: rows, 2: ld, 3: coff, 4: cout}
+    for k, t in enumerate(targets):
+        for slot, word in ((16 + 2 * k, t & 0xffffffff), (17 + 2 * k, (t >> 32) & 0xffffffff)):
+            i[slot] = word - (1 << 32) if word >= (1 << 31) else word
+    return L.make_op(L.OP_SET_BASES, L.F32, p=[None, None, None, None, table.data_ptr()], i=i)
+
+
+def direct_ops(ops):
+    out = []
+    for op in ops:
+        if op.kind == L.OP_CONV and op.i[20] == 2 and op.i[30] == 1:
+            c = L.OmniOp.from_buffer_copy(op)
+            c.i[30] = 0
+            c.p[7] = None
+            op = c
+        out.append(op)
+    return out
 
 
 class PlanBuilder:
@@ -223,7 +245,7 @@
 
     def conv(self, x: View, w_packed: torch.Tensor, bias: Optional[torch.Tensor], out: View, k: int, s: int = 1,
              p: Optional[int] = None, act: int = L.ACT_NONE, res: Optional[View] = None, scale: float = 0.0,
-             out_split: bool = False):
+             out_split: bool = False, base_word: Optional[torch.Tensor] = None):
         p = k // 2 if p is None else p
         Ho = (x.H + 2 * p - k) // s + 1
         Wo = (x.W + 2 * p - k) // s + 1
@@ -259,16 +281,20 @@
         tune = (0, 0)
         if wfmt == 1 and self.conv_tuning:
             tune = tuple(self.conv_tuning.get(conv_key(x.B * Ho * Wo, cout, k * k * x.C, k, s), (0, 0)))
+        if base_word is not None:
+            assert wfmt == 2 and act == L.ACT_NONE and res is None and not out_split, "indirect output base: the LDS-DMA GEMM's plain f32 epilogue"
+            assert base_word.dtype == torch.int64 and base_word.numel() == 1 and base_word.device.type == self.device.type
+            self.keep.append(base_word)
         op = L.make_op(
             L.OP_CONV, self.dtype,
             p=[x.ptr, w_packed.data_ptr(), b.data_ptr() if b is not None else None,
                res.ptr if res is not None else None, out.ptr, self.ws.data_ptr() if self.ws is not None else None,
-               cnt.data_ptr() if cnt is not None else None],
+               cnt.data_ptr() if cnt is not None else None, base_word.data_ptr() if base_word is not None else None],
             i={0: x.B, 1: x.H, 2: x.W, 3: x.C, 4: x.ld, 5: x.coff, 6: k, 7: k, 8: s, 9: p, 10: Ho, 11: Wo,
                12: cout, 13: out.ld, 14: out.coff, 15: act,
                16: res.ld if res is not None else 0, 17: res.coff if res is not None else 0,
                19: self.ws_kib if self.ws is not None else 0, 20: wfmt, 21: 1 if out_split else 0,
-               22: tune[0], 23: tune[1], 24: cnt.numel() if cnt is not None else 0},
+               22: tune[0], 23: tune[1], 24: cnt.numel() if cnt is not None else 0, 30: 1 if base_word is not None else 0},
             f={0: scale, 1: getattr(w_packed, "omni_oscale", 0.0) if wfmt == 2 else 0.0})
         self.ops.append(op)
         self.keep.append(w_packed)
@@ -372,7 +398,8 @@
         t.omni_fmt = 1
         return t
 
-    def conv_patch(self, x: View, w_patch: torch.Tensor, bias: torch.Tensor, out: View, k: int, s: int, p: int, act: int = L.ACT_NONE):
+    def conv_patch(self, x: View, w_patch: torch.Tensor, bias: torch.Tensor, out: View, k: int, s: int, p: int, act: int = L.ACT_NONE,
+                   ln=None, tile: int = 0, splits: int = 0):
         assert self.dtype == L.F32 and x.fmt == "f32" and x.ld == 4 and x.coff == 0 and x.C == 4 and k <= 8
         Ho = (x.H + 2 * p - k) // s + 1
         Wo = (x.W + 2 * p - k) // s + 1
@@ -381,17 +408,34 @@
         assert bias.device.type == self.device.type and bias.dtype == torch.float32 and bias.numel() == cout
         if self.ws is None and (self.device.type == "cuda" or self.workspace_on_host):
             self.ws = self.raw((self.ws_kib * 256,), torch.float32, zero=False)
+        pl, il, fl = [], {}, {}
+        if ln is not None:
+            g, b, eps = ln
+            assert all(t.device.type == self.device.type and t.dtype == torch.float32 and t.numel() == cout for t in (g, b))
+            pl, il, fl = [g.data_ptr(), b.data_ptr()], {31: 1}, {2: eps}
+            self.keep += [g, b]
         self.ops.append(L.make_op(
             L.OP_CONV, self.dtype,
-            p=[x.ptr, w_patch.data_ptr(), bias.data_ptr(), None, out.ptr, self.ws.data_ptr() if self.ws is not None else None],
+            p=[x.ptr, w_patch.data_ptr(), bias.data_ptr(), None, out.ptr, self.ws.data_ptr() if self.ws is not None else None] + pl,
             i={0: x.B, 1: x.H, 2: x.W, 3: 32, 4: 4, 5: 0, 6: k, 7: 1, 8: s, 9: p, 10: Ho, 11: Wo, 12: cout, 13: out.ld, 14: out.coff,
-               15: act, 19: self.ws_kib if self.ws is not None else 0, 20: 1, 25: 1}))
+               15: act, 19: self.ws_kib if self.ws is not None else 0, 20: 1, 22: tile, 23: splits, 25: 1, **il}, f=fl))
         self.keep += [w_patch, bias]
         out.fmt = "f32"
         M = x.B * Ho * Wo
         self.flops += 2 * M * cout * k * k * x.C
         self.bytes += 4 * (x.B * x.H * x.W * x.C + cout * k * k * x.C + M * cout)
         return out
+
+    def patch_fuses_ln(self, x: View, cout: int, k: int, s: int, p: int) -> bool:
+        if self.dtype != L.F32 or cout != 128:
+            return False
+        Ho, Wo = (x.H + 2 * p - k) // s + 1, (x.W + 2 * p - k) // s + 1
+        ws = self.ws is not None or self.device.type == "cuda" or self.workspace_on_host
+        op = L.make_op(L.OP_CONV, self.dtype, p=[256, 256, 256, None, 256, 256 if ws else None],
+                       i={0: x.B, 1: x.H, 2: x.W, 3: 32, 4: 4, 5: 0, 6: k, 7: 1, 8: s, 9: p, 10: Ho, 11: Wo, 12: cout, 13: cout, 14: 0,
+                          19: self.ws_kib if ws else 0, 20: 1, 25: 1})
+        cfg = L.conv_cfg(op)
+        return (cfg["bm"], cfg["bn"], cfg["splits"]) == (128, 128, 1)
 
     def mlp_fused(self, x: View, w1: torch.Tensor, b1: torch.Tensor, w2: torch.Tensor, b2: torch.Tensor, res: View, out: View):
         C, hid = x.C, b1.numel()
```
